# raimis/torchmd-net

Measured on AMD Instinct MI355X. Metric: molecules/sec (energy+force) ET-QM9, higher is better.
Workload: dtype fp32; 1 GPU; ET-QM9 energy+forces (TorchMD_Net derivative=True); model=equivariant-transformer, embedding_dimension=128, num_layers=8, num_rbf=64, num_heads=8, molecules_per_gpu=32, atoms_per_gpu=678, global_batch=32, parallelism=dp1, execution=hip-graph replay

## Files before the change

include/tmdnet.h:

```cpp
#ifndef TMDNET_H
#define TMDNET_H
#include <stddef.h>
#include <stdint.h>

#ifdef __cplusplus
extern "C" {
#endif

enum { TMDNET_OK = 0, TMDNET_BAD_ARGUMENT = 1, TMDNET_UNSUPPORTED = 2, TMDNET_LAUNCH_FAILED = 3,
       TMDNET_WORKSPACE_TOO_SMALL = 4 };
enum { TMDNET_F32 = 0, TMDNET_F64 = 1 };
enum { TMDNET_NL_BRUTE = 0, TMDNET_NL_SHARED = 1, TMDNET_NL_CELL = 2 };
enum { TMDNET_RBF_EXPNORM = 0, TMDNET_RBF_GAUSS = 1 };
enum { TMDNET_ACC_VEC_RESIDUAL = 1, TMDNET_ACC_EDGE = 2 };
enum { TMDNET_ACC_GRADS = 32 };
enum { TMDNET_ET_V_PLANAR = 4 };
enum { TMDNET_BWD2_ACC_EDGE = 8, TMDNET_BWD2_ACC_GVEC = 16 };
enum { TMDNET_ET_TWO_PASS = 64 };
enum { TMDNET_ACT_SILU = 0, TMDNET_ACT_SSP = 1, TMDNET_ACT_TANH = 2, TMDNET_ACT_SIGMOID = 3 };
#define TMDNET_ET_ACT(kv, attn) (((kv) << 8) | ((attn) << 12))

size_t tmdnet_nl_workspace_bytes(int n_atoms, int strategy, const double* box9, double cutoff_upper);
int tmdnet_nl_build(int dtype, int strategy, const void* pos, const int64_t* batch, int n_atoms,
                    const double* box9, int use_periodic, double cutoff_lower, double cutoff_upper,
                    int max_pairs, int loop, int include_transpose, int32_t* neighbors, void* deltas,
                    void* distances, int32_t* num_pairs, int32_t* row_ptr, int32_t* transpose_map,
                    int pad_output, void* workspace, size_t workspace_bytes, void* stream);
int tmdnet_nl_build_paired(int dtype, int strategy, const void* pos, const int64_t* batch, int n_atoms,
                           const double* box9, int use_periodic, double cutoff_lower, double cutoff_upper,
                           int max_pairs, int loop, int include_transpose, int32_t* neighbors, void* deltas,
                           void* distances, int32_t* num_pairs, int32_t* row_ptr, int32_t* transpose_map,
                           int pad_output, void* workspace, size_t workspace_bytes, int32_t* pair_row,
                           int32_t* pair_edge, int n_pair_slots, void* stream);

int tmdnet_nl_backward(int dtype, int n_atoms, const int32_t* row_ptr, const int32_t* transpose_map,
                       int max_pairs, const void* grad_deltas, const void* grad_distances,
                       const void* deltas, const void* distances, void* grad_pos, void* stream);
int tmdnet_nl_backward_multi(int dtype, int n_atoms, const int32_t* row_ptr, const int32_t* transpose_map,
                             int max_pairs, const void* grad_deltas, const void* grad_distances,
                             const void* grad_distances2, const void* deltas, const void* distances,
                             void* grad_pos, void* stream);

int tmdnet_nl_backward_edges(int dtype, int n_atoms, const int32_t* neighbors, int max_pairs,
                             const void* grad_deltas, const void* grad_distances, const void* deltas,
                             const void* distances, void* grad_pos, void* stream);

int tmdnet_nl_backward2(int dtype, int n_atoms, const int32_t* row_ptr, const int32_t* src,
                        const int32_t* transpose_map, int max_pairs, const void* grad_distances,
                        const void* deltas, const void* distances, const void* gg_pos, void* d_pos,
                        void* d_grad_deltas, void* d_grad_distances, void* stream);

int tmdnet_edge_geom_fwd(int dtype, int n_edges, int num_rbf, int rbf_type, const int32_t* src,
                         const int32_t* dst, const void* deltas, const void* dist, const void* mu,
                         const void* beta, double cutoff_lower, double cutoff_upper, void* rbf,
                         void* cutoff, void* unit, void* stream);
int tmdnet_edge_geom_fwd_rows(int dtype, int n_edges, int num_rbf, int rbf_type, const int32_t* src,
                              const int32_t* dst, const void* deltas, const void* dist, const void* mu,
                              const void* beta, double cutoff_lower, double cutoff_upper, void* rbf,
                              void* cutoff, void* unit, const int32_t* rows, int n_rows, void* rbf_rows,
                              void* stream);
int tmdnet_edge_geom_fwd_rows2(int dtype, int n_edges, int num_rbf, int rbf_type, const int32_t* src,
                               const int32_t* dst, const void* deltas, const void* dist, const void* mu,
                               const void* beta, double cutoff_lower, double cutoff_upper, void* rbf,
                               void* cutoff, void* unit, const int32_t* rows, int n_rows, void* rbf_rows,
                               void* drbf_rows, void* stream);
int tmdnet_edge_geom_bwd2(int dtype, int n_edges, int num_rbf, int rbf_type, const int32_t* src,
                          const int32_t* dst, const void* deltas, const void* dist, const void* mu,
                          const void* beta, double cutoff_lower, double cutoff_upper,
                          const void* grad_rbf, const void* grad_cutoff, const void* grad_unit,
                          const void* gg_deltas, const void* gg_dist, void* d_grad_rbf,
                          void* d_grad_cutoff, void* d_grad_unit, void* d_dist, void* d_deltas,
                          void* stream);
int tmdnet_rbf_deriv(int dtype, int num_rbf, int rbf_type, const void* dist, const void* mu,
                     const void* beta, double cutoff_lower, double cutoff_upper, const int32_t* rows,
                     int n_rows, void* out, void* stream);
int tmdnet_edge_geom_bwd(int dtype, int n_edges, int num_rbf, int rbf_type, const int32_t* src,
                         const int32_t* dst, const void* deltas, const void* dist, const void* mu,
                         const void* beta, double cutoff_lower, double cutoff_upper,
                         const void* grad_rbf, const void* grad_cutoff, const void* grad_unit,
                         void* grad_dist, void* grad_deltas, void* stream);
int tmdnet_edge_geom_bwd_multi(int dtype, int n_edges, int num_rbf, int rbf_type, const int32_t* src,
                               const int32_t* dst, const void* deltas, const void* dist, const void* mu,
                               const void* beta, double cutoff_lower, double cutoff_upper, const void* grad_rbf,
                               const void* grad_rbf2, const void* grad_rbf3, const void* grad_cutoff,
                               const void* grad_cutoff2, const void* grad_cutoff3, const void* grad_unit,
                               void* grad_dist, void* grad_deltas, void* stream);

int tmdnet_et_message_fwd(int dtype, int n_nodes, int hidden, int heads, const int32_t* row_ptr,
                          const int32_t* src, int max_pairs, const void* q, int ld_q, const void* k,
                          int ld_k, const void* v, int ld_v, const void* vec_in, const void* pk,
                          int ld_pk, const void* pv, int ld_pv, const void* cutoff, const void* unit,
                          void* x_out, void* vec_out, int flags, const int32_t* pk_rows,
                          const int32_t* order, void* stream);
#define TMDNET_TUNE_ET_BOTH_MAX_NODES 1
#define TMDNET_TUNE_ET_MERGED_MIN_NODES 2
int tmdnet_set_tuning(int key, int value);

int tmdnet_et_message_bwd(int dtype, int n_nodes, int hidden, int heads, const int32_t* row_ptr,
                          const int32_t* src, int max_pairs, const void* q, int ld_q, const void* k,
                          int ld_k, const void* v, int ld_v, const void* vec_in, const void* pk,
                          int ld_pk, const void* pv, int ld_pv, const void* cutoff, const void* unit,
// ... 150 lines not shown
#define TMDNET_TN_POST_O3 1
#define TMDNET_TN_POST_SO3 2
#define TMDNET_TN_RESID 3
#define TMDNET_TN_NORMS 4
#define TMDNET_TN_ENORM 5
#define TMDNET_TN_EOUT 6
int tmdnet_tn_node_fwd(int dtype, int op, int n_nodes, int hidden, const void* a, const void* b,
                       void* out, void* stream);
int tmdnet_tn_node_bwd(int dtype, int op, int n_nodes, int hidden, const void* a, const void* b,
                       const void* grad_out, const void* grad_add, void* ga, void* gb,
                       void* stream);
int tmdnet_tn_node_bwd2(int dtype, int op, int n_nodes, int hidden, const void* a, const void* b,
                        const void* grad_out, const void* t_a, const void* t_b, void* d_grad_out, void* d_a,
                        void* d_b, void* stream);

int tmdnet_silu_fwd(int dtype, int rows, int cols, const void* x, int ld_x, const void* row_scale,
                    void* out, void* stream);
int tmdnet_silu_bwd(int dtype, int rows, int cols, const void* x, int ld_x, const void* row_scale,
                    const void* grad_out, int ld_g, void* grad_x, void* grad_scale, void* stream);
int tmdnet_mlp2_up(int dtype, int rows, int cols, const void* pre, int ld_pre, const void* ghat, const void* a,
                   int ld_a, const void* gy, const void* scale, const void* sbar, void* ahat, void* dpre, void* dgy,
                   void* dscale, void* stream);
int tmdnet_mlp2_down(int dtype, int rows, int cols, const void* pre, int ld_pre, const void* dh, const void* dp,
                     void* c, void* stream);

int tmdnet_atom_sum_fwd(int dtype, int n_atoms, int n_mol, const void* x, const int64_t* batch,
                        const void* std_, const void* mean, void* y, void* stream);
int tmdnet_atom_sum_bwd(int dtype, int n_atoms, int n_mol, const void* grad_y, const int64_t* batch,
                        const void* std_, void* grad_x, void* stream);

int tmdnet_dot_sum_fwd(int dtype, int n_atoms, int K, const void* h, int ld_h, const void* w, const void* b0,
                       int n_mol, const int64_t* batch, const void* std_, const void* mean, void* y, void* stream);
int tmdnet_dot_sum_bwd(int dtype, int n_atoms, int K, const void* grad_y, const int64_t* batch, int n_mol,
                       const void* std_, const void* w, void* grad_h, void* stream);
int tmdnet_dot_sum_fwd_atoms(int dtype, int n_atoms, int K, const void* h, int ld_h, const void* w, const void* b0,
                             int n_mol, const int64_t* batch, const void* std_, const void* mean, void* atom_buf,
                             void* y, void* stream);

int tmdnet_layernorm_fwd_f32(int rows, int C, const void* x, int ldx, const void* w, const void* b, double eps,
                             void* y, int ldy, void* mean, void* rstd, void* stream);
int tmdnet_layernorm_bwd_f32(int rows, int C, const void* x, int ldx, const void* w, const void* mean,
                             const void* rstd, const void* grad_y, int ldg, void* grad_x, int accumulate,
                             void* stream);
int tmdnet_layernorm_bwd2_f32(int rows, int C, const void* x, int ldx, const void* w, const void* mean,
                              const void* rstd, const void* grad_y, int ldg, const void* t_gx, const void* t_gw,
                              const void* t_gb, void* d_grad_y, void* d_x, void* t_row, void* stream);
size_t tmdnet_layernorm_wgrad_workspace_bytes(int rows, int C);
int tmdnet_layernorm_wgrad_f32(int rows, int C, const void* x, int ldx, const void* mean, const void* rstd,
                               const void* grad_y, int ldg, void* grad_w, void* grad_b, void* workspace,
                               size_t workspace_bytes, void* stream);

size_t tmdnet_pair_index_workspace_bytes(int n_nodes);
int tmdnet_pair_index(int n_nodes, const int32_t* row_ptr, const int32_t* src, const int32_t* dst,
                      const int32_t* transpose, int max_pairs, const int32_t* num_pairs, int sorted_rows,
                      int32_t* pair_row, int32_t* pair_edge, int n_pair_slots, void* workspace,
                      size_t workspace_bytes, void* stream);

int tmdnet_gemm_f32(int n_problems, const int* dims, const void* const* ptrs, void* stream);
int tmdnet_gemm_ex_f32(int n_problems, const int* dims, const void* const* ptrs, void* stream);
int tmdnet_gemm_tn_f32(int n_problems, const int* dims, const void* const* ptrs, void* stream);
size_t tmdnet_gemm_tn_workspace_bytes(int n_problems, const int* dims);
int tmdnet_gemm_tn_f32_ws(int n_problems, const int* dims, const void* const* ptrs, void* workspace,
                          size_t workspace_bytes, void* stream);
int tmdnet_gemm_tn_rows_f32_ws(int n_problems, const int* dims, const void* const* ptrs, void* workspace,
                               size_t workspace_bytes, void* stream);
int tmdnet_embedding_fwd_f32(int n, int H, int num_types, const int64_t* z, int n_tables,
                             const void* const* tables, const int* ld_tables, void* const* outs,
                             const int* ld_outs, void* stream);
int tmdnet_embedding_bwd_f32(int n, int H, int num_types, const int64_t* z, int n_tables,
                             const void* const* grads, const int* ld_grads, void* const* outs, int accumulate,
                             void* stream);
int tmdnet_split_t_f32(int N, int K, const void* B, int ldb, void* Bp, void* stream);
int tmdnet_gemm_x3_f32(int M, int N, int K, const void* A, int lda, const void* Bp, const void* bias, void* C,
                       int ldc, int beta, void* stream);
int tmdnet_gemm_x3_ex_f32(int M, int N, int K, const void* A, int lda, const void* Bp, const void* bias, void* C,
                          int ldc, int beta, int act, void* pre, const void* rscale, const void* dpre, int ldx,
                          void* stream);
int tmdnet_gemm_x3w_f32(int M, int N, int K, const void* A, int lda, const void* W, int ldw, int trans_w,
                        const void* bias, void* C, int ldc, int beta, int act, void* pre, const void* rscale,
                        const void* dpre, int ldx, void* stream);
int tmdnet_proj_split_f32(int N, int K, const void* W, int ldw, void* Wp, void* stream);
int tmdnet_proj_f32(int M, int N, int K, const void* A, int lda, const void* Wp, long long piece_stride,
                    const void* bias, void* C, int ldc, void* stream);

size_t tmdnet_fep_image_bytes(int D, int R);
int tmdnet_fep_split_f32(int D, int R, const void* W, int ldw, const void* bias, void* img, void* wsc,
                         void* bias_out, void* stream);
size_t tmdnet_fep_frags_bytes(long long rows, int R);
int tmdnet_fep_frags_f32(long long rows, int R, const void* r_rows, const void* mu, const void* beta,
                         double cutoff_lower, double cutoff_upper, int rbf_type, void* frags, void* dscale,
                         void* stream);
int tmdnet_et_fused_fwd_f32(int n_nodes, int hidden, int heads, int num_rbf, const int32_t* row_ptr,
                            const int32_t* src, int max_pairs, const void* q, int ld_q, const void* k, int ld_k,
                            const void* v, int ld_v, const void* vec_in, const void* cutoff, const void* unit,
                            const int32_t* frag_rows, const void* frags, long long n_frag_rows, const void* img,
                            const void* wsc, const void* bias, void* x_out, void* vec_out, int flags, void* stream);

size_t tmdnet_et_fused_bwd_workspace_bytes(int max_pairs);
int tmdnet_et_fused_bwd_f32(int n_nodes, int hidden, int heads, int num_rbf, const int32_t* row_ptr,
                            const int32_t* src, int max_pairs, const void* q, int ld_q, const void* k, int ld_k,
                            const void* v, int ld_v, const void* vec_in, const void* cutoff, const void* unit,
                            const int32_t* frag_rows, const void* frags, const void* dscale, long long n_frag_rows,
                            const void* img, const void* wsc, const void* bias, const void* grad_x,
                            const void* grad_vec, void* gq, void* gk, void* gv, void* gvec_in, void* gcut,
                            void* gunit, void* gdist, int accumulate, void* workspace, size_t workspace_bytes,
                            void* stream);

int tmdnet_nbr_fused_fwd_f32(int n_nodes, int hidden, int num_rbf, const int32_t* row_ptr, const int32_t* src,
                             int max_pairs, const void* x, int ld_x, const void* cutoff, const int32_t* frag_rows,
                             const void* frags, long long n_frag_rows, const void* img, const void* wsc,
                             const void* bias, void* out, int ld_out, const void* x_self, void* out_self,
                             void* stream);
int tmdnet_nbr_fused_bwd_f32(int n_nodes, int hidden, int num_rbf, const int32_t* row_ptr, const int32_t* src,
                             int max_pairs, const void* x, int ld_x, const void* cutoff, const int32_t* frag_rows,
                             const void* frags, const void* dscale, long long n_frag_rows, const void* img,
                             const void* wsc, const void* bias, const void* grad_out, int ld_grad_out, void* gcut,
                             void* gdist, int accumulate, void* stream);

int tmdnet_mse2_fwd(int dtype, int n1, const void* a1, const void* b1, double w1, int n2, const void* a2,
                    const void* b2, double w2, void* out, void* stream);
int tmdnet_mse2_bwd(int dtype, int n1, const void* a1, const void* b1, double w1, int n2, const void* a2,
                    const void* b2, double w2, const void* grad_out, void* d1, void* d2, void* stream);

const char* tmdnet_build_info(void);

#ifdef __cplusplus
}
#endif
#endif
```

torchmd-net_amd/csrc/et_message.hip:

```cpp
#include <cstdlib>

#include "common.h"
#include "tmdnet.h"

namespace tmd {
namespace et {

template <typename T, int V> struct Vec;
template <> struct Vec<float, 1> { using t = float; };
template <> struct Vec<float, 2> { using t = float2; };
template <> struct Vec<float, 4> { using t = float4; };
template <> struct Vec<double, 1> { using t = double; };
template <> struct Vec<double, 2> { using t = double2; };
template <> struct Vec<double, 4> { using t = double4; };

template <typename T, int V> __device__ __forceinline__ void ldv(T (&o)[V], const T* p);
template <typename T, int V> __device__ __forceinline__ void ldv_(T (&o)[V], const T* p) {
  using VT = typename Vec<T, V>::t;
  const VT x = *reinterpret_cast<const VT*>(p);
  if constexpr (V == 1) { o[0] = x; }
  else if constexpr (V == 2) { o[0] = x.x; o[1] = x.y; }
  else { o[0] = x.x; o[1] = x.y; o[2] = x.z; o[3] = x.w; }
}
template <typename T, int V> __device__ __forceinline__ void ldv(T (&o)[V], const T* p) {
// ... 20 lines not shown
  if constexpr (V == 8) {
    T a[4], b[4];
#pragma unroll
    for (int i = 0; i < 4; ++i) { a[i] = o[i]; b[i] = o[4 + i]; }
    stv_<T, 4>(p, a);
    stv_<T, 4>(p + 4, b);
  } else {
    stv_<T, V>(p, o);
  }
}
template <typename T, int V> __device__ __forceinline__ void stv_acc(T* p, const T (&o)[V], bool acc) {
  if (acc) {
    T q[V];
    ldv<T, V>(q, p);
#pragma unroll
    for (int i = 0; i < V; ++i) q[i] += o[i];
    stv<T, V>(p, q);
  } else {
    stv<T, V>(p, o);
  }
}
template <typename T, int V> __device__ __forceinline__ void zero(T (&o)[V]) {
#pragma unroll
  for (int i = 0; i < V; ++i) o[i] = T(0);
}

template <typename T> struct Args {
  int n, H, d, L, lph, cap;
  int xcd;
  int HC;
  const int32_t* row_ptr;
  const int32_t* src;
  const int32_t* order;
  const T* q; int ldq;
  const T* k; int ldk;
  const T* v; int ldv;
  const T* vec;
  const T* pk; int ldpk;
  const T* pv; int ldpv;
  const int32_t* prow;
  const T* dpk;
  const T* dpv;
  T* gr;
  const T* C;
  const T* u;
  T* xo; T* veco;
  const T* gx; const T* gvec;
  T* gq; T* gk; T* gv; T* gveci; T* gpk; T* gpv; T* gC; T* gu;
  int acc;
  int planar;
  int vst;
  int act_kv;
  int act_at;
};

template <typename T, int V>
__device__ __forceinline__ void act(const T (&x)[V], bool has, T (&s)[V], T (&ds)[V], int code) {
  if (code == kActSilu) {
#pragma unroll
    for (int i = 0; i < V; ++i) {
      if (has) {
        Silu<T> f(x[i]);
        s[i] = f.s;
        ds[i] = f.d(x[i]);
      } else {
        s[i] = T(1);
        ds[i] = T(0);
      }
    }
    return;
  }
#pragma unroll
  for (int i = 0; i < V; ++i) {
    if (has) {
      ActF<T> f(x[i], code);
      s[i] = f.s;
      ds[i] = f.d(x[i]);
    } else {
      s[i] = T(1);
      ds[i] = T(0);
    }
  }
}
template <typename T> __device__ __forceinline__ const T* opt(const T* p, size_t off, const T* dummy) {
  return p ? p + off : dummy;
}


__device__ __forceinline__ int xcd_block(int b, int nwg, int xcd) { return xcd ? xcd_remap(b, nwg) : b; }
struct Geo {
  int node;
  int sub;
  int es;
  int el;
  int cg;
};

template <int S, int CS, bool ORD, int WPB = 4>
__device__ __forceinline__ Geo geo(int n, int L, const int32_t* order, int xcd, int blk, int nwg) {
  Geo g;
  const int wid = threadIdx.x >> 6;
  const int npb = WPB / S;
  const int nbn = (n + npb - 1) / npb;
  const int lb = xcd_block(blk, nwg, xcd);
  g.cg = CS > 1 ? __builtin_amdgcn_readfirstlane(lb / nbn) : 0;
  const int w = __builtin_amdgcn_readfirstlane((CS > 1 ? lb % nbn : lb) * npb + wid / S);
  g.sub = __builtin_amdgcn_readfirstlane(wid % S);
  g.node = w < n ? (ORD ? __builtin_amdgcn_readfirstlane(order[w]) : w) : -1;
  const int lane = lane_id();
  g.es = lane / L;
  g.el = lane % L;
  return g;
}

template <typename T, int V> __device__ __forceinline__ void xor_slots(T (&a)[V], int L) {
  for (int o = L; o < TMD_WAVE; o <<= 1)
#pragma unroll
    for (int i = 0; i < V; ++i) a[i] += __shfl_xor(a[i], o);
}

template <typename T, int S, int NV>
__device__ __forceinline__ void reduce_waves(T (&a)[NV], int sub, T* lds) {
  if constexpr (S > 1) {
    const int wid = threadIdx.x >> 6, lane = lane_id();
    const int base = (wid - sub) * 64 * NV;
    if (sub > 0) {
#pragma unroll
      for (int i = 0; i < NV; ++i) lds[base + (sub * NV + i) * 64 + lane] = a[i];
    }
    __syncthreads();
    if (sub == 0) {
#pragma unroll
      for (int s2 = 1; s2 < S; ++s2)
#pragma unroll
        for (int i = 0; i < NV; ++i) a[i] += lds[base + (s2 * NV + i) * 64 + lane];
    }
  }
}

template <typename T, int S, int PD, typename St, typename LD, typename F>
__device__ __forceinline__ void edge_chunks_pf(const Args<T>& A, int b, int e, int EPW, const Geo& G,
                                               LD&& ld, F&& body) {
  const int lane = lane_id();
  St cur, nxt, nx2;
  const int step = EPW * S;
  for (int c = b; c < e; c += TMD_WAVE) {
    const int n = min(TMD_WAVE, e - c);
    int s_r = 0, p_r = c + lane;
    T C_r = T(0), u0_r = T(0), u1_r = T(0), u2_r = T(0);
    if (lane < n) {
      const int k = c + lane;
      s_r = A.src[k];
      TMD_DCHECK(s_r >= 0 && s_r < A.n);
      if (A.prow) p_r = A.prow[k];
      C_r = A.C[k];
      u0_r = A.u[3 * k];
      u1_r = A.u[3 * k + 1];
      u2_r = A.u[3 * k + 2];
    }
    int j0 = EPW * G.sub;
    if (j0 < n) {
      ld(__shfl(p_r, min(j0 + G.es, n - 1)), cur);
      if constexpr (PD == 2) ld(__shfl(p_r, min(j0 + step + G.es, n - 1)), nxt);
    }
    for (; j0 < n; j0 += step) {
      const int j = j0 + G.es;
      const int jj = j < n ? j : n - 1;
      const int s = __shfl(s_r, jj);
      const T Ce = __shfl(C_r, jj), u0 = __shfl(u0_r, jj), u1 = __shfl(u1_r, jj), u2 = __shfl(u2_r, jj);
      const int kn = __shfl(p_r, min(j0 + PD * step + G.es, n - 1));
      auto pre = [&]() { ld(kn, PD == 2 ? nx2 : nxt); };
      if (j < n) body(c + j, s, Ce, u0, u1, u2, cur, pre);
      else pre();
      cur = nxt;
      if constexpr (PD == 2) nxt = nx2;
    }
  }
}

template <typename T, int S, typename F>
__device__ __forceinline__ void edge_chunks(const Args<T>& A, int b, int e, int EPW, const Geo& G, F&& body) {
  const int lane = lane_id();
  const int step = EPW * S;
  for (int c = b; c < e; c += TMD_WAVE) {
    const int n = min(TMD_WAVE, e - c);
    int s_r = 0, p_r = c + lane;
    T C_r = T(0), u0_r = T(0), u1_r = T(0), u2_r = T(0);
    if (lane < n) {
      const int k = c + lane;
      s_r = A.src[k];
      TMD_DCHECK(s_r >= 0 && s_r < A.n);
      if (A.prow) p_r = A.prow[k];
      C_r = A.C[k];
      u0_r = A.u[3 * k];
      u1_r = A.u[3 * k + 1];
      u2_r = A.u[3 * k + 2];
    }
    for (int j0 = EPW * G.sub; j0 < n; j0 += step) {
      const int j = j0 + G.es;
      const int jj = j < n ? j : n - 1;
      const int s = __shfl(s_r, jj), row = __shfl(p_r, jj);
      const T Ce = __shfl(C_r, jj), u0 = __shfl(u0_r, jj), u1 = __shfl(u1_r, jj), u2 = __shfl(u2_r, jj);
      if (j < n) body(c + j, s, Ce, u0, u1, u2, row);
    }
  }
}

template <typename T, int V, int S, int CS, bool ORD, bool GA = true>
__global__ __launch_bounds__(256) void k_fwd(Args<T> A) {
  const int AKV = GA ? A.act_kv : kActSilu, AAT = GA ? A.act_at : kActSilu;
  __shared__ T lds[S > 1 ? 4 * 64 * 4 * V : 1];
  const Geo G = geo<S, CS, ORD>(A.n, A.L, A.order, A.xcd, blockIdx.x, gridDim.x);
  const int t = G.node;
  const bool on = true;
  const int EPW = TMD_WAVE / A.L;
  const int c0 = G.cg * A.HC + G.el * V;
  const int hh = c0 / A.d, cc = c0 % A.d;
  const int vo = A.planar ? c0 : hh * 3 * A.d + cc;
  const bool hk = A.pk != nullptr, hv = A.pv != nullptr, hw = A.vec != nullptr;
  const int pvd = hv ? A.vst : 0, vcd = hw ? A.H : 0;
  (void)vcd;
  T ax[V], a0[V], a1[V], a2[V];
  zero(ax); zero(a0); zero(a1); zero(a2);
  if (t >= 0) {
    T q[V];
    ldv<T, V>(q, A.q + (size_t)t * A.ldq + c0);
    const int b = min(A.row_ptr[t], A.cap), e = min(A.row_ptr[t + 1], A.cap);
    const T* dummy = A.q + (size_t)t * A.ldq;
    struct St { T k[V], x[V], a[V], b[V]; };
    auto ld = [&](int k, St& st) {
      ldv<T, V>(st.k, opt(A.pk, (size_t)k * A.ldpk + c0, dummy + c0));
      const T* pvs = opt(A.pv, (size_t)k * A.ldpv + vo, dummy);
      ldv<T, V>(st.x, pvs);
      ldv<T, V>(st.a, pvs + pvd);
      ldv<T, V>(st.b, pvs + 2 * pvd);
    };
    auto body = [&](int k, int s, T Ce, T u0, T u1, T u2, const St& st, auto&& pre) {
      (void)k;
      T kk[V], vx[V], v1[V], v2[V], w0[V], w1[V], w2[V];
      ldv<T, V>(kk, A.k + (size_t)s * A.ldk + c0);
      const T* vs = A.v + (size_t)s * A.ldv + vo;
      ldv<T, V>(vx, vs);
      ldv<T, V>(v1, vs + A.vst);
      ldv<T, V>(v2, vs + 2 * A.vst);
      const T* vecs = hw ? A.vec + (size_t)s * 3 * A.H + c0 : dummy + c0;
      ldv<T, V>(w0, vecs);
      ldv<T, V>(w1, vecs + vcd);
      ldv<T, V>(w2, vecs + 2 * vcd);
      pre();
      if (!hw) { zero(w0); zero(w1); zero(w2); }
      T dk[V], dvx[V], dv1[V], dv2[V], dd[V];
      act<T, V>(st.k, hk, dk, dd, AKV);
      act<T, V>(st.x, hv, dvx, dd, AKV);
      act<T, V>(st.a, hv, dv1, dd, AKV);
      act<T, V>(st.b, hv, dv2, dd, AKV);
      T part = T(0);
#pragma unroll
      for (int i = 0; i < V; ++i) part += q[i] * kk[i] * dk[i];
      part = group_sum(part, A.lph);
      const ActF<T> sa(part, AAT);
      const T a = sa.s * Ce;
#pragma unroll
      for (int i = 0; i < V; ++i) {
        ax[i] += vx[i] * dvx[i] * a;
        const T v1e = v1[i] * dv1[i], v2e = v2[i] * dv2[i];
        a0[i] += w0[i] * v1e + v2e * u0;
        a1[i] += w1[i] * v1e + v2e * u1;
        a2[i] += w2[i] * v1e + v2e * u2;
      }
    };
    edge_chunks_pf<T, S, 1, St>(A, b, e, EPW, G, ld, body);
  }
  xor_slots(ax, A.L); xor_slots(a0, A.L); xor_slots(a1, A.L); xor_slots(a2, A.L);
  T all[4 * V];
#pragma unroll
  for (int i = 0; i < V; ++i) { all[i] = ax[i]; all[V + i] = a0[i]; all[2 * V + i] = a1[i]; all[3 * V + i] = a2[i]; }
  reduce_waves<T, S, 4 * V>(all, G.sub, lds);
  if (t >= 0 && G.sub == 0 && on && G.es == 0) {
#pragma unroll
    for (int i = 0; i < V; ++i) { ax[i] = all[i]; a0[i] = all[V + i]; a1[i] = all[2 * V + i]; a2[i] = all[3 * V + i]; }
    stv<T, V>(A.xo + (size_t)t * A.H + c0, ax);
    T* vo_ = A.veco + (size_t)t * 3 * A.H + c0;
    stv<T, V>(vo_, a0);
    stv<T, V>(vo_ + A.H, a1);
    stv<T, V>(vo_ + 2 * A.H, a2);
  }
}

template <typename T>
__device__ __forceinline__ void zero_pad_rows(const Args<T>& A, int blk, int nwg) {
  const int e0 = min(A.row_ptr[A.n], A.cap);
  if (e0 >= A.cap) return;
  const long long rows = A.cap - e0;
  const long long tid = (long long)blk * blockDim.x + threadIdx.x, nth = (long long)nwg * blockDim.x;
  if (A.gpk) {
    for (long long i = tid; i < rows * A.H; i += nth)
      A.gpk[(size_t)(e0 + i / A.H) * A.ldpk + i % A.H] = T(0);
  }
  if (A.gpv) {
    const int w = 3 * A.H;
    for (long long i = tid; i < rows * w; i += nth)
      A.gpv[(size_t)(e0 + i / w) * A.ldpv + i % w] = T(0);
  }
  if (A.gC)
    for (long long i = tid; i < rows; i += nth) A.gC[e0 + i] = T(0);
  if (A.gu)
    for (long long i = tid; i < rows * 3; i += nth) A.gu[3 * (size_t)e0 + i] = T(0);
  if (A.gr)
    for (long long i = tid; i < rows; i += nth) A.gr[e0 + i] = T(0);
}

template <typename T, int V, int S, int CS, bool DR, bool AG = false, bool GA = true>
__device__ __forceinline__ void bwd_dst_body(const Args<T>& A, int blk, int nwg) {
  const int AKV = GA ? A.act_kv : kActSilu, AAT = GA ? A.act_at : kActSilu;
  __shared__ T lds[S > 1 ? 4 * 64 * V : 1];
  const Geo G = geo<S, CS, false>(A.n, A.L, nullptr, A.xcd, blk, nwg);
  const int t = G.node;
  const bool on = true;
  const int EPW = TMD_WAVE / A.L;
  const int c0 = G.cg * A.HC + G.el * V;
  const int hh = c0 / A.d, cc = c0 % A.d;
  const int vo = A.planar ? c0 : hh * 3 * A.d + cc;
  const bool hk = A.pk != nullptr, hv = A.pv != nullptr, hw = A.vec != nullptr;
  const int pvd = hv ? A.vst : 0, vcd = hw ? A.H : 0;
  (void)vcd;
  const bool head_leader = on && (G.el % A.lph) == 0;
  T gq[V];
  zero(gq);
  if (t >= 0) {
    T q[V], gx[V], g0[V], g1[V], g2[V];
    ldv<T, V>(q, A.q + (size_t)t * A.ldq + c0);
    ldv<T, V>(gx, A.gx + (size_t)t * A.H + c0);
    const T* gvt = A.gvec + (size_t)t * 3 * A.H + c0;
    ldv<T, V>(g0, gvt);
    ldv<T, V>(g1, gvt + A.H);
    ldv<T, V>(g2, gvt + 2 * A.H);
    const int b = min(A.row_ptr[t], A.cap), e = min(A.row_ptr[t + 1], A.cap);
    const T* dummy = A.q + (size_t)t * A.ldq;
    const bool acc_edge = (A.acc & TMDNET_ACC_EDGE) && G.el == 0;
    struct St { T k[V], x[V], a[V], b[V]; int row; };
    auto ld = [&](int k, St& st) {
      ldv<T, V>(st.k, opt(A.pk, (size_t)k * A.ldpk + c0, dummy + c0));
      const T* pvs = opt(A.pv, (size_t)k * A.ldpv + vo, dummy);
      ldv<T, V>(st.x, pvs);
      ldv<T, V>(st.a, pvs + pvd);
      ldv<T, V>(st.b, pvs + 2 * pvd);
      st.row = k;
    };
    auto body = [&](int k, int s, T Ce, T u0, T u1, T u2, const St& st, auto&& pre) {
      T oc = T(0), ou0 = T(0), ou1 = T(0), ou2 = T(0), orr = T(0);
      if (acc_edge) {
        oc = A.gC[k];
        ou0 = A.gu[3 * k];
        ou1 = A.gu[3 * k + 1];
        ou2 = A.gu[3 * k + 2];
        if constexpr (DR) orr = A.gr[k];
      }
      T kk[V], vx[V], v1[V], v2[V], w0[V], w1[V], w2[V];
      ldv<T, V>(kk, A.k + (size_t)s * A.ldk + c0);
      const T* vs = A.v + (size_t)s * A.ldv + vo;
      ldv<T, V>(vx, vs);
      ldv<T, V>(v1, vs + A.vst);
      ldv<T, V>(v2, vs + 2 * A.vst);
      const T* vecs = hw ? A.vec + (size_t)s * 3 * A.H + c0 : dummy + c0;
      ldv<T, V>(w0, vecs);
      ldv<T, V>(w1, vecs + vcd);
      ldv<T, V>(w2, vecs + 2 * vcd);
      T ik[AG ? V : 1], ix[AG ? V : 1], i1[AG ? V : 1], i2[AG ? V : 1];
      if constexpr (AG) {
        if (hk) ldv<T, V>(ik, A.gpk + (size_t)k * A.ldpk + c0); else zero(ik);
        if (hv) {
          const T* gp = A.gpv + (size_t)k * A.ldpv + vo;
          ldv<T, V>(ix, gp); ldv<T, V>(i1, gp + A.vst); ldv<T, V>(i2, gp + 2 * A.vst);
        } else {
          zero(ix); zero(i1); zero(i2);
        }
      }
      T dpk_[DR ? V : 1], dpx_[DR ? V : 1], dp1_[DR ? V : 1], dp2_[DR ? V : 1];
      if constexpr (DR) {
        ldv<T, V>(dpk_, opt(A.dpk, (size_t)st.row * A.ldpk + c0, dummy + c0));
        const T* dps = opt(A.dpv, (size_t)st.row * A.ldpv + vo, dummy);
        ldv<T, V>(dpx_, dps);
        ldv<T, V>(dp1_, dps + pvd);
        ldv<T, V>(dp2_, dps + 2 * pvd);
      }
      pre();
      if (!hw) { zero(w0); zero(w1); zero(w2); }
      const T (&pk)[V] = st.k;
      const T (&px)[V] = st.x;
      const T (&p1)[V] = st.a;
      const T (&p2)[V] = st.b;
      T dk[V], ddk[V], dvx[V], dv1[V], dv2[V], ddx[V], dd1[V], dd2[V];
      act<T, V>(pk, hk, dk, ddk, AKV);
      act<T, V>(px, hv, dvx, ddx, AKV);
      act<T, V>(p1, hv, dv1, dd1, AKV);
      act<T, V>(p2, hv, dv2, dd2, AKV);
      T part = T(0), ga = T(0), gu0 = T(0), gu1 = T(0), gu2 = T(0);
#pragma unroll
      for (int i = 0; i < V; ++i) {
        part += q[i] * kk[i] * dk[i];
        ga += gx[i] * vx[i] * dvx[i];
        const T v2e = v2[i] * dv2[i];
        gu0 += g0[i] * v2e;
        gu1 += g1[i] * v2e;
        gu2 += g2[i] * v2e;
      }
      part = group_sum(part, A.lph);
      ga = group_sum(ga, A.lph);
      const ActF<T> sa(part, AAT);
      const T a = sa.s * Ce;
      const T gs = ga * Ce * sa.d(part);
      T gpk[V], gpx[V], gp1[V], gp2[V];
#pragma unroll
      for (int i = 0; i < V; ++i) {
        gq[i] += gs * kk[i] * dk[i];
        gpk[i] = gs * q[i] * kk[i] * ddk[i];
        gpx[i] = gx[i] * a * vx[i] * ddx[i];
        const T gv1e = g0[i] * w0[i] + g1[i] * w1[i] + g2[i] * w2[i];
        gp1[i] = gv1e * v1[i] * dd1[i];
        const T gv2e = g0[i] * u0 + g1[i] * u1 + g2[i] * u2;
        gp2[i] = gv2e * v2[i] * dd2[i];
      }
      const T gc = group_sum(head_leader ? ga * sa.s : T(0), A.L);
      gu0 = group_sum(gu0, A.L);
      gu1 = group_sum(gu1, A.L);
      gu2 = group_sum(gu2, A.L);
      T grr = T(0);
      if constexpr (DR) {
#pragma unroll
        for (int i = 0; i < V; ++i)
          grr += (hk ? gpk[i] * dpk_[i] : T(0)) +
                 (hv ? gpx[i] * dpx_[i] + gp1[i] * dp1_[i] + gp2[i] * dp2_[i] : T(0));
        grr = group_sum(grr, A.L);
        if (on && (A.gpk || A.gpv)) {
          if (hk && A.gpk) stv<T, V>(A.gpk + (size_t)k * A.ldpk + c0, gpk);
          if (hv && A.gpv) {
            T* gp = A.gpv + (size_t)k * A.ldpv + vo;
            stv<T, V>(gp, gpx);
            stv<T, V>(gp + A.vst, gp1);
            stv<T, V>(gp + 2 * A.vst, gp2);
          }
        }
      } else {
        if (on) {
          if constexpr (AG) {
#pragma unroll
            for (int i = 0; i < V; ++i) { gpk[i] += ik[i]; gpx[i] += ix[i]; gp1[i] += i1[i]; gp2[i] += i2[i]; }
          }
          const bool ag = !AG && (A.acc & TMDNET_ACC_GRADS);
          if (hk) stv_acc<T, V>(A.gpk + (size_t)k * A.ldpk + c0, gpk, ag);
          if (hv) {
            T* gp = A.gpv + (size_t)k * A.ldpv + vo;
            stv_acc<T, V>(gp, gpx, ag);
            stv_acc<T, V>(gp + A.vst, gp1, ag);
            stv_acc<T, V>(gp + 2 * A.vst, gp2, ag);
          }
        }
      }
      if (G.el == 0) {
        A.gC[k] = oc + gc;
        A.gu[3 * k] = ou0 + gu0;
        A.gu[3 * k + 1] = ou1 + gu1;
        A.gu[3 * k + 2] = ou2 + gu2;
        if constexpr (DR) A.gr[k] = orr + grr;
      }
    };
    edge_chunks_pf<T, S, 1, St>(A, b, e, EPW, G, ld, body);
  }
  xor_slots(gq, A.L);
  reduce_waves<T, S, V>(gq, G.sub, lds);
  if (t >= 0 && G.sub == 0 && on && G.es == 0)
    stv_acc<T, V>(A.gq + (size_t)t * A.ldq + c0, gq, A.acc & TMDNET_ACC_GRADS);
  zero_pad_rows(A, blk, nwg);
}

template <typename T, int V, int S, int CS, bool GA = true>
__device__ __forceinline__ void bwd_src_body(const Args<T>& A, int blk, int nwg) {
  const int AKV = GA ? A.act_kv : kActSilu, AAT = GA ? A.act_at : kActSilu;
  __shared__ T lds[S > 1 ? 4 * 64 * 7 * V : 1];
  const Geo G = geo<S, CS, false>(A.n, A.L, nullptr, A.xcd, blk, nwg);
  const int j = G.node;
  const bool on = true;
  const int EPW = TMD_WAVE / A.L;
  const int c0 = G.cg * A.HC + G.el * V;
  const int hh = c0 / A.d, cc = c0 % A.d;
  const int vo = A.planar ? c0 : hh * 3 * A.d + cc;
  const bool hk = A.pk != nullptr, hv = A.pv != nullptr, hw = A.vec != nullptr;
  const int pvd = hv ? A.vst : 0, vcd = hw ? A.H : 0;
  (void)vcd;
  T gk[V], gvx[V], gv1[V], gv2[V], gw0[V], gw1[V], gw2[V];
  zero(gk); zero(gvx); zero(gv1); zero(gv2); zero(gw0); zero(gw1); zero(gw2);
  if (j >= 0) {
    T kk[V], vx[V], v1[V], v2[V], w0[V], w1[V], w2[V];
    ldv<T, V>(kk, A.k + (size_t)j * A.ldk + c0);
    const T* vj = A.v + (size_t)j * A.ldv + vo;
    ldv<T, V>(vx, vj);
    ldv<T, V>(v1, vj + A.vst);
    ldv<T, V>(v2, vj + 2 * A.vst);
    if (hw) {
      const T* vecj = A.vec + (size_t)j * 3 * A.H + c0;
      ldv<T, V>(w0, vecj);
      ldv<T, V>(w1, vecj + A.H);
      ldv<T, V>(w2, vecj + 2 * A.H);
    } else {
      zero(w0); zero(w1); zero(w2);
    }
    const int b = min(A.row_ptr[j], A.cap), e = min(A.row_ptr[j + 1], A.cap);
    const T* dummy = A.k + (size_t)j * A.ldk;
    struct St { T k[V], x[V], a[V], b[V]; };
    auto ld = [&](int k, St& st) {
      ldv<T, V>(st.k, opt(A.pk, (size_t)k * A.ldpk + c0, dummy + c0));
      const T* pvs = opt(A.pv, (size_t)k * A.ldpv + vo, dummy);
      ldv<T, V>(st.x, pvs);
      ldv<T, V>(st.a, pvs + pvd);
      ldv<T, V>(st.b, pvs + 2 * pvd);
    };
    auto body = [&](int k, int m, T Ce, T u0, T u1, T u2, const St& st, auto&& pre) {
      u0 = -u0; u1 = -u1; u2 = -u2;
      (void)k;
      T qm[V], gxm[V], g0[V], g1[V], g2[V];
      ldv<T, V>(qm, A.q + (size_t)m * A.ldq + c0);
      ldv<T, V>(gxm, A.gx + (size_t)m * A.H + c0);
      const T* gvm = A.gvec + (size_t)m * 3 * A.H + c0;
      ldv<T, V>(g0, gvm);
      ldv<T, V>(g1, gvm + A.H);
      ldv<T, V>(g2, gvm + 2 * A.H);
      pre();
      const T (&pk)[V] = st.k;
      const T (&px)[V] = st.x;
      const T (&p1)[V] = st.a;
      const T (&p2)[V] = st.b;
      T dk[V], ddk[V], dvx[V], dv1[V], dv2[V], dd[V];
      act<T, V>(pk, hk, dk, ddk, AKV);
      act<T, V>(px, hv, dvx, dd, AKV);
      act<T, V>(p1, hv, dv1, dd, AKV);
      act<T, V>(p2, hv, dv2, dd, AKV);
      T part = T(0), ga = T(0);
#pragma unroll
      for (int i = 0; i < V; ++i) {
        part += qm[i] * kk[i] * dk[i];
        ga += gxm[i] * vx[i] * dvx[i];
      }
      part = group_sum(part, A.lph);
      ga = group_sum(ga, A.lph);
      const ActF<T> sa(part, AAT);
      const T a = sa.s * Ce;
      const T gs = ga * Ce * sa.d(part);
#pragma unroll
      for (int i = 0; i < V; ++i) {
        gk[i] += gs * qm[i] * dk[i];
        gvx[i] += gxm[i] * a * dvx[i];
        const T gv1e = g0[i] * w0[i] + g1[i] * w1[i] + g2[i] * w2[i];
        gv1[i] += gv1e * dv1[i];
        const T gv2e = g0[i] * u0 + g1[i] * u1 + g2[i] * u2;
        gv2[i] += gv2e * dv2[i];
        const T v1e = v1[i] * dv1[i];
        gw0[i] += g0[i] * v1e;
        gw1[i] += g1[i] * v1e;
        gw2[i] += g2[i] * v1e;
      }
    };
    edge_chunks_pf<T, S, 1, St>(A, b, e, EPW, G, ld, body);
  }
  xor_slots(gk, A.L); xor_slots(gvx, A.L); xor_slots(gv1, A.L); xor_slots(gv2, A.L); xor_slots(gw0, A.L); xor_slots(gw1, A.L); xor_slots(gw2, A.L);
  T all[7 * V];
#pragma unroll
  for (int i = 0; i < V; ++i) {
    all[i] = gk[i]; all[V + i] = gvx[i]; all[2 * V + i] = gv1[i]; all[3 * V + i] = gv2[i];
    all[4 * V + i] = gw0[i]; all[5 * V + i] = gw1[i]; all[6 * V + i] = gw2[i];
  }
  reduce_waves<T, S, 7 * V>(all, G.sub, lds);
  if (j >= 0 && G.sub == 0 && on && G.es == 0) {
#pragma unroll
    for (int i = 0; i < V; ++i) {
      gk[i] = all[i]; gvx[i] = all[V + i]; gv1[i] = all[2 * V + i]; gv2[i] = all[3 * V + i];
      gw0[i] = all[4 * V + i]; gw1[i] = all[5 * V + i]; gw2[i] = all[6 * V + i];
    }
    const bool ag = A.acc & TMDNET_ACC_GRADS;
    stv_acc<T, V>(A.gk + (size_t)j * A.ldk + c0, gk, ag);
    T* gvj = A.gv + (size_t)j * A.ldv + vo;
    stv_acc<T, V>(gvj, gvx, ag);
    stv_acc<T, V>(gvj + A.vst, gv1, ag);
    stv_acc<T, V>(gvj + 2 * A.vst, gv2, ag);
    if (A.gveci != nullptr) {
      if (A.acc & TMDNET_ACC_VEC_RESIDUAL) {
        const T* gr = A.gvec + (size_t)j * 3 * A.H + c0;
        T r0[V], r1[V], r2[V];
        ldv<T, V>(r0, gr);
        ldv<T, V>(r1, gr + A.H);
        ldv<T, V>(r2, gr + 2 * A.H);
#pragma unroll
        for (int i = 0; i < V; ++i) { gw0[i] += r0[i]; gw1[i] += r1[i]; gw2[i] += r2[i]; }
      }
      T* gwj = A.gveci + (size_t)j * 3 * A.H + c0;
      stv_acc<T, V>(gwj, gw0, ag);
      stv_acc<T, V>(gwj + A.H, gw1, ag);
      stv_acc<T, V>(gwj + 2 * A.H, gw2, ag);
    }
  }
}

template <typename T, int V, bool DR>
constexpr int bwd_min_waves() { return (DR && sizeof(T) == 4 && V <= 4) ? 3 : 1; }

template <typename T, int V, int S, int CS, bool DR, bool AG = false, bool GA = true>
__global__ __launch_bounds__(256, (bwd_min_waves<T, V, DR>())) void k_bwd_dst(Args<T> A) {
  bwd_dst_body<T, V, S, CS, DR, AG, GA>(A, blockIdx.x, gridDim.x);
}
template <typename T, int V, int S, int CS, bool GA = true>
__global__ __launch_bounds__(256) void k_bwd_src(Args<T> A) {
  bwd_src_body<T, V, S, CS, GA>(A, blockIdx.x, gridDim.x);
}
template <typename T, int V, int S, int CS, bool DR, bool AG = false, bool GA = true>
__global__ __launch_bounds__(256, (bwd_min_waves<T, V, DR>())) void k_bwd_both(Args<T> A) {
  const int split = (int)gridDim.x / 2;
  if ((int)blockIdx.x < split) bwd_dst_body<T, V, S, CS, DR, AG, GA>(A, blockIdx.x, split);
  else bwd_src_body<T, V, S, CS, GA>(A, blockIdx.x - split, split);
}

template <typename T, int V, int S, int PD, bool GA = true>
__device__ __forceinline__ void bwd_merged_body(const Args<T>& A, int blk, int nwg) {
  const int AKV = GA ? A.act_kv : kActSilu, AAT = GA ? A.act_at : kActSilu;
  constexpr int NA = 8 * V;
  extern __shared__ __attribute__((aligned(16))) char dyn_lds[];
  T* lds = reinterpret_cast<T*>(dyn_lds);
  const int HM = A.H;
  const Geo G = geo<S, 1, false>(A.n, A.L, nullptr, A.xcd, blk, nwg);
  const int t = G.node;
  const int EPW = TMD_WAVE / A.L;
  const int c0 = G.el * V;
  const int hh = c0 / A.d, cc = c0 % A.d;
  const int vo = A.planar ? c0 : hh * 3 * A.d + cc;
  const bool hk = A.pk != nullptr, hv = A.pv != nullptr, hw = A.vec != nullptr;
  const int pvd = hv ? A.vst : 0, vcd = hw ? A.H : 0;
  const bool head_leader = (G.el % A.lph) == 0;
  T* nv = lds + ((threadIdx.x >> 6) / S) * 12 * HM;
  if (t >= 0 && G.sub == 0 && G.es == 0) {
    T a[V];
    const T* src[12];
    const T* gvt = A.gvec + (size_t)t * 3 * A.H;
    const T* vt = A.v + (size_t)t * A.ldv;
    const T* wt = A.vec + (size_t)t * 3 * A.H;
    src[0] = A.q + (size_t)t * A.ldq + c0; src[1] = A.gx + (size_t)t * A.H + c0;
    src[2] = gvt + c0; src[3] = gvt + A.H + c0; src[4] = gvt + 2 * A.H + c0;
    src[5] = A.k + (size_t)t * A.ldk + c0;
    src[6] = vt + vo; src[7] = vt + vo + A.vst; src[8] = vt + vo + 2 * A.vst;
    src[9] = hw ? wt + c0 : src[0]; src[10] = hw ? wt + A.H + c0 : src[0]; src[11] = hw ? wt + 2 * A.H + c0 : src[0];
#pragma unroll
    for (int r = 0; r < 12; ++r) {
      ldv<T, V>(a, src[r]);
      if (r >= 9 && !hw) zero(a);
      stv<T, V>(nv + r * HM + c0, a);
    }
  }
  __syncthreads();
  T gq[V], gk[V], gvx[V], gv1[V], gv2[V], gw0[V], gw1[V], gw2[V];
  zero(gq); zero(gk); zero(gvx); zero(gv1); zero(gv2); zero(gw0); zero(gw1); zero(gw2);
  if (t >= 0) {
    const int b = min(A.row_ptr[t], A.cap), e = min(A.row_ptr[t + 1], A.cap);
    const T* dummy = A.q + (size_t)t * A.ldq;
    const bool acc_edge = (A.acc & TMDNET_ACC_EDGE) && G.el == 0;
    struct St { T k[V], x[V], a[V], b[V]; int row; };
    auto ld = [&](int k, St& st) {
      ldv<T, V>(st.k, opt(A.pk, (size_t)k * A.ldpk + c0, dummy + c0));
      const T* pvs = opt(A.pv, (size_t)k * A.ldpv + vo, dummy);
      ldv<T, V>(st.x, pvs);
      ldv<T, V>(st.a, pvs + pvd);
      ldv<T, V>(st.b, pvs + 2 * pvd);
      st.row = k;
    };
    auto body = [&](int k, int s, T Ce, T u0, T u1, T u2, const St& st, auto&& pre) {
      T oc = T(0), ou0 = T(0), ou1 = T(0), ou2 = T(0), orr = T(0);
      if (acc_edge) {
        oc = A.gC[k]; ou0 = A.gu[3 * k]; ou1 = A.gu[3 * k + 1]; ou2 = A.gu[3 * k + 2]; orr = A.gr[k];
      }
      T kk[V], vx[V], v1[V], v2[V], w0[V], w1[V], w2[V], qs[V], gxs[V], h0[V], h1[V], h2[V];
      ldv<T, V>(kk, A.k + (size_t)s * A.ldk + c0);
      const T* vs = A.v + (size_t)s * A.ldv + vo;
      ldv<T, V>(vx, vs);
      ldv<T, V>(v1, vs + A.vst);
      ldv<T, V>(v2, vs + 2 * A.vst);
      const T* vecs = hw ? A.vec + (size_t)s * 3 * A.H + c0 : dummy + c0;
      ldv<T, V>(w0, vecs);
      ldv<T, V>(w1, vecs + vcd);
      ldv<T, V>(w2, vecs + 2 * vcd);
      ldv<T, V>(qs, A.q + (size_t)s * A.ldq + c0);
      ldv<T, V>(gxs, A.gx + (size_t)s * A.H + c0);
      const T* gvs = A.gvec + (size_t)s * 3 * A.H + c0;
      ldv<T, V>(h0, gvs);
      ldv<T, V>(h1, gvs + A.H);
      ldv<T, V>(h2, gvs + 2 * A.H);
      T dpk_[V], dpx_[V], dp1_[V], dp2_[V];
      ldv<T, V>(dpk_, opt(A.dpk, (size_t)st.row * A.ldpk + c0, dummy + c0));
      const T* dps = opt(A.dpv, (size_t)st.row * A.ldpv + vo, dummy);
      ldv<T, V>(dpx_, dps);
      ldv<T, V>(dp1_, dps + pvd);
      ldv<T, V>(dp2_, dps + 2 * pvd);
      pre();
      if (!hw) { zero(w0); zero(w1); zero(w2); }
      T dk[V], ddk[V], dvx[V], dv1[V], dv2[V], ddx[V], dd1[V], dd2[V];
// ... 608 lines not shown
    if (A.dC) {
#pragma unroll
      for (int u = 0; u < NB_U; ++u) dc[u] = wave_sum(on ? dc[u] : T(0));
      if (lane == 0) {
#pragma unroll
        for (int u = 0; u < NB_U; ++u)
          if (sq[u] >= 0) A.dC[k0 + u] = dc[u];
      }
    }
  });
  if (on && A.dgout) stv<T, V>(A.dgout + (size_t)t * A.H + c0, acc);
}

template <typename T, int V>
__global__ __launch_bounds__(256) void k_nb_bwd2_src(NbArgs<T> A) {
  const int j = blockIdx.x * (blockDim.x / TMD_WAVE) + threadIdx.x / TMD_WAVE;
  if (j >= A.n) return;
  const int lane = lane_id();
  const bool on = lane < A.L;
  const int c0 = on ? lane * V : 0;
  T acc[V];
  zero(acc);
  nb_edges(A, j, [&](int k0, const int (&sq)[NB_U], const T (&cq)[NB_U]) {
    T gm[NB_U][V], wk[NB_U][V], gwk[NB_U][V], ck[NB_U], gck[NB_U];
#pragma unroll
    for (int u = 0; u < NB_U; ++u) {
      const int kt = sq[u] >= 0 ? A.tr[k0 + u] : -1;
      const bool live = kt >= 0 && sq[u] != j;
      const int m = live ? sq[u] : j;
      const int k = live ? kt : k0;
      TMD_DCHECK(!live || k < A.cap);
      ldv<T, V>(gm[u], A.gout + (size_t)m * A.ldg + c0);
      ldv<T, V>(wk[u], A.w + (size_t)k * A.ldw + c0);
      if (A.ggw) ldv<T, V>(gwk[u], A.ggw + (size_t)k * A.H + c0); else zero(gwk[u]);
      ck[u] = live ? A.C[k] : T(0);
      gck[u] = (live && A.ggC) ? A.ggC[k] : T(0);
    }
#pragma unroll
    for (int u = 0; u < NB_U; ++u)
#pragma unroll
      for (int i = 0; i < V; ++i) acc[i] += gm[u][i] * (gwk[u][i] * ck[u] + gck[u] * wk[u][i]);
  });
  if (on) stv<T, V>(A.dx + (size_t)j * A.H + c0, acc);
}

static inline int pick_vec(int H) {
  if (H % 256 == 0) return 4;
  if (H % 128 == 0) return 2;
  return 1;
}

template <typename T>
static bool aligned(const void* p, int ld, int V) {
  if (!p) return true;
  return ((uintptr_t)p % (sizeof(T) * V)) == 0 && (ld % V) == 0;
}

template <typename T, template <typename, int> class K, typename AT>
static int launch_v(int V, int n, AT A, hipStream_t st) {
  const int tb = 256, wpb = tb / TMD_WAVE;
  dim3 g((n + wpb - 1) / wpb);
  if (n <= 0) return kOk;
  if (V == 1) hipLaunchKernelGGL((K<T, 1>::fn), g, dim3(tb), 0, st, A);
  else if (V == 2) hipLaunchKernelGGL((K<T, 2>::fn), g, dim3(tb), 0, st, A);
  else hipLaunchKernelGGL((K<T, 4>::fn), g, dim3(tb), 0, st, A);
  return hipGetLastError() == hipSuccess ? kOk : kLaunchFailed;
}

static inline int et_waves_per_node(int n, int bytes_per_lane_vec) {
  if (bytes_per_lane_vec > 32) return 1;
  static const int env_s = [] { const char* e = getenv("TMDNET_ET_S"); return e ? atoi(e) : 0; }();
  if (env_s > 0) return env_s >= 4 ? 4 : env_s >= 2 ? 2 : 1;
  if (n < 4096) return 4;
  if (n < 8192) return 2;
  return 1;
}

template <typename T, int V, int S, int KIND, bool ORD, bool GA>
static int et_launch_k(const Args<T>& A, dim3 g, dim3 b, int nbn, hipStream_t st);

template <typename T, int V, int S, int KIND, bool ORD>
static int et_launch_vs(Args<T> A, hipStream_t st) {
  int cs = 1;
  if (KIND == 1 || A.H % (cs * V) || (A.H / cs / V) & (A.H / cs / V - 1) || A.H / cs / V < A.lph ||
      A.H / cs / V > 64)
    cs = 1;
  A.HC = A.H / cs;
  A.L = A.HC / V;
  if (A.L > 64 || (A.L & (A.L - 1))) return kUnsupported;
  const int nbn = (A.n + (4 / S) - 1) / (4 / S);
  const dim3 g(nbn * cs), b(256);
  if (A.act_kv == kActSilu && A.act_at == kActSilu)
    return et_launch_k<T, V, S, KIND, ORD, false>(A, g, b, nbn, st);
  return et_launch_k<T, V, S, KIND, ORD, true>(A, g, b, nbn, st);
}

template <typename T, int V, int S, int KIND, bool ORD, bool GA>
static int et_launch_k(const Args<T>& A, dim3 g, dim3 b, int nbn, hipStream_t st) {
  if (KIND == 0) hipLaunchKernelGGL((k_fwd<T, V, S, 1, ORD, GA>), g, b, 0, st, A);
  else if (KIND == 1) hipLaunchKernelGGL((k_bwd_dst<T, V, S, 1, false, false, GA>), g, b, 0, st, A);
  else if (KIND == 2) hipLaunchKernelGGL((k_bwd_src<T, V, S, 1, GA>), g, b, 0, st, A);
  else if (KIND == 3) hipLaunchKernelGGL((k_bwd_both<T, V, S, 1, false, false, GA>), dim3(2 * nbn), b, 0, st, A);
  else if (KIND == 4) hipLaunchKernelGGL((k_bwd_dst<T, V, S, 1, true, false, GA>), g, b, 0, st, A);
  else if (KIND == 5) hipLaunchKernelGGL((k_bwd_both<T, V, S, 1, true, false, GA>), dim3(2 * nbn), b, 0, st, A);
  else if (KIND == 6) hipLaunchKernelGGL((k_bwd_both<T, V, S, 1, false, true, GA>), dim3(2 * nbn), b, 0, st, A);
  else if (KIND == 8 || KIND == 9) {
    const size_t node = (size_t)(4 / S) * 12 * A.H, red = S > 1 ? 4 * 64 * 8 * V : 1;
    const size_t bytes = (node > red ? node : red) * sizeof(T);
    if (KIND == 8) hipLaunchKernelGGL((k_bwd_merged<T, V, S, 1, GA>), dim3(nbn), b, bytes, st, A);
    else hipLaunchKernelGGL((k_bwd_merged<T, V, S, 0, GA>), dim3(nbn), b, bytes, st, A);
  }
  else hipLaunchKernelGGL((k_bwd_dst<T, V, S, 1, false, true, GA>), g, b, 0, st, A);
  return hipGetLastError() == hipSuccess ? kOk : kLaunchFailed;
}

static constexpr int kBwdFuseNodes = 16384;

static int g_tune[3] = {-1, -1, -1};
static int tune_get(int key) {
  int& v = g_tune[key];
  if (v < 0) {
    const char* e = getenv(key == TMDNET_TUNE_ET_BOTH_MAX_NODES ? "TMDNET_ET_FUSE" : "TMDNET_ET_MERGED_MIN");
    v = e ? atoi(e) : kBwdFuseNodes;
  }
  return v;
}

template <typename T, int V, int KIND, bool ORD>
static int et_launch_v(const Args<T>& A, hipStream_t st) {
  int S = et_waves_per_node(A.n, (int)sizeof(T) * V);
  static const bool env_s_set = getenv("TMDNET_ET_S") != nullptr;
  if (KIND == 0 && !env_s_set && (int)sizeof(T) * V <= 32) S = 4;
  static const int bwd_s = getenv("TMDNET_ET_BWD_S") ? atoi(getenv("TMDNET_ET_BWD_S")) : 0;
  if (KIND != 0 && bwd_s && (int)sizeof(T) * V <= 32) S = bwd_s >= 4 ? 4 : bwd_s >= 2 ? 2 : 1;
  if (S == 4) return et_launch_vs<T, V, (sizeof(T) * V <= 32 ? 4 : 1), KIND, ORD>(A, st);
  if (S == 2) return et_launch_vs<T, V, (sizeof(T) * V <= 32 ? 2 : 1), KIND, ORD>(A, st);
  return et_launch_vs<T, V, 1, KIND, ORD>(A, st);
}

template <typename T, int KIND, bool ORD>
static int et_launch(int V, const Args<T>& A, hipStream_t st) {
  if (A.n <= 0) return kOk;
  switch (V) {
    case 1: return et_launch_v<T, 1, KIND, ORD>(A, st);
    case 2: return et_launch_v<T, 2, KIND, ORD>(A, st);
    case 4: return et_launch_v<T, 4, KIND, ORD>(A, st);
    case 8: return et_launch_v<T, 8, KIND, ORD>(A, st);
  }
  return kUnsupported;
}

template <typename T, int V> struct KNbFwd { static constexpr auto fn = k_nb_fwd<T, V>; };
template <typename T, int V> struct KNbDst { static constexpr auto fn = k_nb_bwd_dst<T, V>; };
template <typename T, int V> struct KNbSrc { static constexpr auto fn = k_nb_bwd_src<T, V>; };
template <typename T, int V> struct KNb2Dst { static constexpr auto fn = k_nb_bwd2_dst<T, V>; };
template <typename T, int V> struct KNb2Src { static constexpr auto fn = k_nb_bwd2_src<T, V>; };

template <typename T>
static int setup(Args<T>& A, int n, int H, int heads, const int32_t* row_ptr, const int32_t* src,
                 int cap, const void* q, int ldq, const void* k, int ldk, const void* v, int ldv_,
                 const void* vec, const void* pk, int ldpk, const void* pv, int ldpv, const void* C,
                 const void* u, const int32_t* order, int& V, const int32_t* prow = nullptr) {
  if (H <= 0 || heads <= 0 || H % heads) return kBadArgument;
  if (H % 32 == 0) V = H / 32;
  else if (H < 32) V = 1;
  else return kUnsupported;

  if (V != 1 && V != 2 && V != 4 && V != 8) return kUnsupported;
  const int d = H / heads;
  if (d % V) return kUnsupported;
  const int lph = d / V;
  if (lph & (lph - 1)) return kUnsupported;
  const int VA = V > 4 ? 4 : V;
  if (!aligned<T>(q, ldq, VA) || !aligned<T>(k, ldk, VA) || !aligned<T>(v, ldv_, VA) ||
      !aligned<T>(pk, ldpk, VA) || !aligned<T>(pv, ldpv, VA) || !aligned<T>(vec, H, VA))
    return kBadArgument;
  A = Args<T>{};
  A.n = n; A.H = H; A.d = d; A.L = H / V; A.HC = H; A.lph = lph; A.cap = cap;
  A.planar = 0; A.vst = d;
  A.row_ptr = row_ptr; A.src = src; A.order = order;
  A.xcd = 1;
  A.q = (const T*)q; A.ldq = ldq; A.k = (const T*)k; A.ldk = ldk; A.v = (const T*)v; A.ldv = ldv_;
  A.vec = (const T*)vec; A.pk = (const T*)pk; A.ldpk = ldpk; A.pv = (const T*)pv; A.ldpv = ldpv;
  A.prow = prow;
  A.C = (const T*)C; A.u = (const T*)u;
  return kOk;
}

template <typename T>
static int set_acts(Args<T>& A, int flags) {
  A.act_kv = (flags >> 8) & 15;
  A.act_at = (flags >> 12) & 15;
  return (A.act_kv > kActSigmoid || A.act_at > kActSigmoid) ? kBadArgument : kOk;
}

template <typename T>
static int fwd(int n, int H, int heads, const int32_t* row_ptr, const int32_t* src, int cap,
               const void* q, int ldq, const void* k, int ldk, const void* v, int ldv_,
               const void* vec, const void* pk, int ldpk, const void* pv, int ldpv, const void* C,
               const void* u, void* xo, void* veco, int flags, const int32_t* prow, const int32_t* order,
               hipStream_t st) {
  Args<T> A;
  int V;
  int rc = setup<T>(A, n, H, heads, row_ptr, src, cap, q, ldq, k, ldk, v, ldv_, vec, pk, ldpk, pv,
                    ldpv, C, u, order, V, prow);
  if (rc) return rc;
  if ((rc = set_acts(A, flags))) return rc;
  if (flags & TMDNET_ET_V_PLANAR) { A.planar = 1; A.vst = H; }
  A.xo = (T*)xo;
  A.veco = (T*)veco;
  return order ? et_launch<T, 0, true>(V, A, st) : et_launch<T, 0, false>(V, A, st);
}

template <typename T>
static int bwd(int n, int H, int heads, const int32_t* row_ptr, const int32_t* src, int cap,
               const void* q, int ldq, const void* k, int ldk, const void* v, int ldv_,
               const void* vec, const void* pk, int ldpk, const void* pv, int ldpv, const void* C,
               const void* u, const void* gx, const void* gvec, void* gq, void* gk, void* gv,
               void* gveci, void* gpk, void* gpv, void* gC, void* gu, const void* dpk, const void* dpv,
               void* gr, int acc, const int32_t* prow, const int32_t* order, hipStream_t st) {
  Args<T> A;
  int V;
  int rc = setup<T>(A, n, H, heads, row_ptr, src, cap, q, ldq, k, ldk, v, ldv_, vec, pk, ldpk, pv,
                    ldpv, C, u, order, V, prow);
  if (rc) return rc;
  A.gx = (const T*)gx; A.gvec = (const T*)gvec;
  A.gq = (T*)gq; A.gk = (T*)gk; A.gv = (T*)gv; A.gveci = (T*)gveci;
  A.gpk = (T*)gpk; A.gpv = (T*)gpv; A.gC = (T*)gC; A.gu = (T*)gu;
  A.dpk = (const T*)dpk; A.dpv = (const T*)dpv; A.gr = (T*)gr;
  A.acc = acc;
  if ((rc = set_acts(A, acc))) return rc;
  static const int bwd_v = getenv("TMDNET_ET_BWD_V") ? atoi(getenv("TMDNET_ET_BWD_V")) : 0;
  if (bwd_v && bwd_v < V && H % (32 * bwd_v) == 0 && H / bwd_v <= 64 && (A.d / bwd_v) > 0 &&
      A.d % bwd_v == 0 && !((A.d / bwd_v) & (A.d / bwd_v - 1))) {
    V = bwd_v;
    A.lph = A.d / V;
  }
  if (acc & TMDNET_ET_V_PLANAR) { A.planar = 1; A.vst = H; }
  const bool dr = gr != nullptr;
  if (dr && ((A.pk && !dpk) || (A.pv && !dpv))) return kBadArgument;
  if (!dr && ((A.pk && !gpk) || (A.pv && !gpv))) return kBadArgument;
  const int fuse_nodes = tune_get(TMDNET_TUNE_ET_BOTH_MAX_NODES);
  const bool ag = !dr && (acc & TMDNET_ACC_GRADS) && (A.pk || A.pv);
  static const int merged = getenv("TMDNET_ET_MERGED") ? atoi(getenv("TMDNET_ET_MERGED")) : 1;
  const int merged_min = tune_get(TMDNET_TUNE_ET_MERGED_MIN_NODES);
  if (dr && merged && n >= merged_min && !(acc & TMDNET_ET_TWO_PASS) && !A.gpk && !A.gpv)
    return merged == 2 ? et_launch<T, 9, false>(V, A, st) : et_launch<T, 8, false>(V, A, st);
  if (n < fuse_nodes)
    return dr ? et_launch<T, 5, false>(V, A, st) : ag ? et_launch<T, 6, false>(V, A, st) : et_launch<T, 3, false>(V, A, st);
  rc = dr ? et_launch<T, 4, false>(V, A, st) : ag ? et_launch<T, 7, false>(V, A, st) : et_launch<T, 1, false>(V, A, st);
  if (rc) return rc;
  return et_launch<T, 2, false>(V, A, st);
}

struct Bwd2Ex {
  int ldggq, ldggk, ldggv, ldoq, ldok, ldov, ldopk, ldopv;
  const int32_t* tr;
  void* scratch;
  const int32_t* prow;
  const void* ggsc;
};

template <typename T>
static int bwd2(int n, int H, int heads, const int32_t* row_ptr, const int32_t* src, int cap,
                const void* q, int ldq, const void* k, int ldk, const void* v, int ldv_,
                const void* vec, const void* pk, int ldpk, const void* pv, int ldpv, const void* C,
                const void* u, const void* gx, const void* gvec, const void* ggq, const void* ggk,
                const void* ggv, const void* ggw, const void* ggpk, int ldggpk, const void* ggpv,
                int ldggpv, const void* ggC, const void* ggu, void* o_gx, void* o_gvec, void* o_q,
                void* o_k, void* o_v, void* o_vec, void* o_pk, void* o_pv, void* o_C, void* o_u,
                int flags, hipStream_t st, const Bwd2Ex* ex = nullptr) {
  Args2<T> B{};
  int V;
  int rc = setup<T>(B.a, n, H, heads, row_ptr, src, cap, q, ldq, k, ldk, v, ldv_, vec, pk, ldpk, pv,
                    ldpv, C, u, nullptr, V);
  if (rc) return rc;
  if (H % 64 == 0) V = H / 64;
  const int d = H / heads;
  if ((V != 1 && V != 2 && V != 4) || d % V || ((d / V) & (d / V - 1))) return kUnsupported;
  B.a.L = H / V;
  B.a.lph = d / V;
  if (B.a.L > 64 || (B.a.L & (B.a.L - 1))) return kUnsupported;
  if (!aligned<T>(ggpk, ldggpk, V) || !aligned<T>(ggpv, ldggpv, V)) return kBadArgument;
  if ((rc = set_acts(B.a, flags))) return rc;
  if (flags & TMDNET_ET_V_PLANAR) { B.a.planar = 1; B.a.vst = H; }
  B.a.gx = (const T*)gx; B.a.gvec = (const T*)gvec;
  B.ggq = (const T*)ggq; B.ggk = (const T*)ggk; B.ggv = (const T*)ggv; B.ggw = (const T*)ggw;
  B.ggpk = (const T*)ggpk; B.ldggpk = ldggpk; B.ggpv = (const T*)ggpv; B.ldggpv = ldggpv;
  B.ggC = (const T*)ggC; B.ggu = (const T*)ggu;
  B.o_gx = (T*)o_gx; B.o_gvec = (T*)o_gvec; B.o_q = (T*)o_q; B.o_k = (T*)o_k; B.o_v = (T*)o_v;
  B.o_vec = (T*)o_vec; B.o_pk = (T*)o_pk; B.o_pv = (T*)o_pv; B.o_C = (T*)o_C; B.o_u = (T*)o_u;
  B.ldggq = B.ldok = B.ldoq = H; B.ldggk = H; B.ldggv = B.ldov = 3 * H; B.ldopk = H; B.ldopv = 3 * H;
  if (ex) {
    auto pick = [](int x, int dflt) { return x ? x : dflt; };
    B.ldggq = pick(ex->ldggq, H); B.ldggk = pick(ex->ldggk, H); B.ldggv = pick(ex->ldggv, 3 * H);
    B.ldoq = pick(ex->ldoq, H); B.ldok = pick(ex->ldok, H); B.ldov = pick(ex->ldov, 3 * H);
    B.ldopk = pick(ex->ldopk, H); B.ldopv = pick(ex->ldopv, 3 * H);
    if (B.ldggq < H || B.ldggk < H || B.ldggv < 3 * H || B.ldoq < H || B.ldok < H || B.ldov < 3 * H ||
        B.ldopk < H || B.ldopv < 3 * H)
      return kBadArgument;
    if (!aligned<T>(ggq, B.ldggq, V) || !aligned<T>(ggk, B.ldggk, V) || !aligned<T>(ggv, B.ldggv, V) ||
        !aligned<T>(o_q, B.ldoq, V) || !aligned<T>(o_pk, B.ldopk, V) || !aligned<T>(o_pv, B.ldopv, V))
      return kBadArgument;
    if ((ex->tr == nullptr) != (ex->scratch == nullptr)) return kBadArgument;
    if (ex->scratch) {
      if (H % 4 || B.ldok % 4 || B.ldov % 4 || ((uintptr_t)o_k % (4 * sizeof(T))) ||
          ((uintptr_t)o_v % (4 * sizeof(T))) || ((uintptr_t)ex->scratch % (4 * sizeof(T))))
        return kBadArgument;
      B.tr = ex->tr;
      B.o_src = (T*)ex->scratch;
    }
    B.a.prow = ex->prow;
    if (ex->ggsc && !ex->prow) return kBadArgument;
    B.ggsc = (const T*)ex->ggsc;
  }
  B.acc_edge = (flags & TMDNET_BWD2_ACC_EDGE) ? 1 : 0;
  B.acc_gvec = (flags & TMDNET_BWD2_ACC_GVEC) ? 1 : 0;
  if (n <= 0) return kOk;
  static const int s_env = getenv("TMDNET_BWD2_S") ? atoi(getenv("TMDNET_BWD2_S")) : 0;
  int S = n < 2048 ? 8 : (n < 4096 ? 4 : (n < 8192 ? 2 : 1));
  if (s_env == 1 || s_env == 2 || s_env == 4 || s_env == 8) S = s_env;
  if (S == 8 && V != 2) S = 4;
  const dim3 g(S == 8 ? n : (n + 4 / S - 1) / (4 / S)), b(S == 8 ? 512 : 256);
#define TMD_L2(VV, SS) hipLaunchKernelGGL((k_bwd2<T, VV, SS>), g, b, 0, st, B)
  if (V == 1) { if (S == 4) TMD_L2(1, 4); else if (S == 2) TMD_L2(1, 2); else TMD_L2(1, 1); }
// ... 227 lines not shown
```

torchmd-net_amd/csrc/gemm.hip:

```cpp
#include <cstdio>
#include <cstdlib>

#include "common.h"
#include "tmdnet.h"

namespace tmd {
namespace gemm {

struct Prob {
  int M, N, K, lda, ldb, ldc, trans_b, beta;
  const float* A;
  const float* B;
  const float* bias;
  float* C;
  int tiles_n, tile0;
  int act, ldx;
  float* pre;
  const float* rscale;
  const float* dpre;
};

struct Group {
  Prob p[4];
  int n;
// ... 633 lines not shown
__global__ __launch_bounds__(256) void k_proj_split(int N, int K, const float* W, int ldw, unsigned short* Wp) {
  const int i = blockIdx.x * 256 + threadIdx.x;
  if (i >= N * K / 4) return;
  const int n = i / (K / 4), k = (i % (K / 4)) * 4;
  const float4 v = *reinterpret_cast<const float4*>(W + (size_t)n * ldw + k);
  const float x[4] = {v.x, v.y, v.z, v.w};
  unsigned h[4], m[4], l[4];
#pragma unroll
  for (int j = 0; j < 4; ++j) split3(x[j], h[j], m[j], l[j]);
  const size_t o = (size_t)n * K + k, ps = (size_t)N * K;
  *reinterpret_cast<uint2*>(Wp + o) = make_uint2((h[0] >> 16) | h[1], (h[2] >> 16) | h[3]);
  *reinterpret_cast<uint2*>(Wp + ps + o) = make_uint2((m[0] >> 16) | m[1], (m[2] >> 16) | m[3]);
  *reinterpret_cast<uint2*>(Wp + 2 * ps + o) = make_uint2((l[0] >> 16) | l[1], (l[2] >> 16) | l[3]);
}

template <int KS, int MB, int BN>
__global__ __launch_bounds__(256) void k_proj_x3(Args P) {
  constexpr int K = 32 * KS, LD = K + 8;
  __shared__ __attribute__((aligned(16))) unsigned short w[3][BN][LD];
  __shared__ __attribute__((aligned(16))) float sb[BN];
  const int lane = threadIdx.x & 63, wave = threadIdx.x >> 6;
  const int n0 = blockIdx.x * BN;
  const int m0 = (blockIdx.y * 4 + wave) * (16 * MB);
  const int nr = min(BN, P.N - n0);
  const int kq = 8 * (lane >> 4);
  float4 ar[MB][KS][2];
#pragma unroll
  for (int mb = 0; mb < MB; ++mb) {
    const float* r = P.A + (size_t)min(m0 + 16 * mb + (lane & 15), P.M - 1) * P.lda + kq;
#pragma unroll
    for (int ks = 0; ks < KS; ++ks) {
      ar[mb][ks][0] = *reinterpret_cast<const float4*>(r + 32 * ks);
      ar[mb][ks][1] = *reinterpret_cast<const float4*>(r + 32 * ks + 4);
    }
  }
  constexpr int CH = K / 8;
  constexpr int NL = (3 * BN * CH + 255) / 256;
  u4 stg[NL];
#pragma unroll
  for (int i = 0; i < NL; ++i) {
    const int c = threadIdx.x + 256 * i;
    const int p = c / (BN * CH), rc = c % (BN * CH), n = rc / CH, k = (rc % CH) * 8;
    if (c < 3 * BN * CH)
      stg[i] = *reinterpret_cast<const u4*>(P.Wp + p * P.pstride + (size_t)min(n0 + n, P.N - 1) * K + k);
  }
#pragma unroll
  for (int i = 0; i < NL; ++i) {
    const int c = threadIdx.x + 256 * i;
    const int p = c / (BN * CH), rc = c % (BN * CH), n = rc / CH, k = (rc % CH) * 8;
    if (c < 3 * BN * CH) *reinterpret_cast<u4*>(&w[p][n][k]) = stg[i];
  }
  if (threadIdx.x < BN) sb[threadIdx.x] = P.bias ? P.bias[min(n0 + (int)threadIdx.x, P.N - 1)] : 0.f;
  bf8 a[MB][KS][3];
#pragma unroll
  for (int mb = 0; mb < MB; ++mb)
#pragma unroll
    for (int ks = 0; ks < KS; ++ks) split8(ar[mb][ks][0], ar[mb][ks][1], a[mb][ks]);
  __syncthreads();
  if (m0 >= P.M) return;
  for (int nb = 0; nb < nr; nb += 16) {
    bf8 b[KS][3];
#pragma unroll
    for (int ks = 0; ks < KS; ++ks)
#pragma unroll
      for (int p = 0; p < 3; ++p)
        b[ks][p] = *reinterpret_cast<const bf8*>(&w[p][nb + (lane & 15)][32 * ks + kq]);
    f4 acc[MB];
#pragma unroll
    for (int mb = 0; mb < MB; ++mb) acc[mb] = f4{0.f, 0.f, 0.f, 0.f};
    constexpr int TW[6] = {2, 1, 0, 1, 0, 0}, TA[6] = {0, 1, 2, 0, 1, 0};
#pragma unroll
    for (int t = 0; t < 6; ++t)
#pragma unroll
      for (int ks = 0; ks < KS; ++ks)
#pragma unroll
        for (int mb = 0; mb < MB; ++mb)
          acc[mb] = __builtin_amdgcn_mfma_f32_16x16x32_bf16(b[ks][TW[t]], a[mb][ks][TA[t]], acc[mb], 0, 0, 0);
    const int nl = nb + 4 * (lane >> 4);
    const f4 bv = *reinterpret_cast<const f4*>(&sb[nl]);
#pragma unroll
    for (int mb = 0; mb < MB; ++mb) {
      const int m = m0 + 16 * mb + (lane & 15);
      if (m < P.M) *reinterpret_cast<f4*>(P.C + (size_t)m * P.ldc + n0 + nl) = acc[mb] + bv;
    }
  }
}

__global__ __launch_bounds__(256) void k_split_t(int N, int K, const float* B, int ldb, unsigned short* Bp) {
  const int i = blockIdx.x * 256 + threadIdx.x;
  if (i >= N * (K / 4)) return;
  const int k = (i / N) * 4, n = i % N;
  const float x[4] = {B[(size_t)k * ldb + n], B[(size_t)(k + 1) * ldb + n], B[(size_t)(k + 2) * ldb + n],
                      B[(size_t)(k + 3) * ldb + n]};
  unsigned h[4], m[4], l[4];
#pragma unroll
  for (int j = 0; j < 4; ++j) split3(x[j], h[j], m[j], l[j]);
  const size_t o = (size_t)n * K + k, ps = (size_t)N * K;
  *reinterpret_cast<uint2*>(Bp + o) = make_uint2((h[0] >> 16) | h[1], (h[2] >> 16) | h[3]);
  *reinterpret_cast<uint2*>(Bp + ps + o) = make_uint2((m[0] >> 16) | m[1], (m[2] >> 16) | m[3]);
  *reinterpret_cast<uint2*>(Bp + 2 * ps + o) = make_uint2((l[0] >> 16) | l[1], (l[2] >> 16) | l[3]);
}

struct XArgs {
  int M, N, K, lda, ldc, beta;
  int nx, ny, remap;
  const float* A;
  const unsigned short* Bp;
  const float* bias;
  float* C;
  int act, ldx;
  float* pre;
  const float* rscale;
  const float* dpre;
  const float* W;
  int ldw;
};
template <int MB, int BN, int PD, int WS = 0>
__global__ __launch_bounds__(256) void k_gemm_x3(XArgs P) {
  constexpr int KC = BN >= 128 ? 64 : 128, LD = KC + 8, NB = BN / 16, SPC = KC / 32;
  __shared__ __attribute__((aligned(16))) unsigned short w[3][BN][LD];
  const int lane = threadIdx.x & 63, wave = threadIdx.x >> 6;
  int bx = blockIdx.x, by = blockIdx.y;
  if (P.remap) {
    const int T = P.nx * P.ny, b = blockIdx.x, x = b & 7, q = T >> 3, r = T & 7;
    const int t = x * q + min(x, r) + (b >> 3);
    bx = t % P.nx;
    by = t / P.nx;
  }
  const int n0 = bx * BN;
  const int m0 = (by * 4 + wave) * (16 * MB);
  const int kq = 8 * (lane >> 4);
  const size_t ps = (size_t)P.N * P.K;
  f4 acc[NB][MB];
#pragma unroll
  for (int nb = 0; nb < NB; ++nb)
#pragma unroll
    for (int mb = 0; mb < MB; ++mb) acc[nb][mb] = f4{0.f, 0.f, 0.f, 0.f};
  const float* arow[MB];
#pragma unroll
  for (int mb = 0; mb < MB; ++mb) arow[mb] = P.A + (size_t)min(m0 + 16 * mb + (lane & 15), P.M - 1) * P.lda + kq;
  const int nks_all = P.K / 32;
  float4 an[PD][MB][2];
#pragma unroll
  for (int d = 0; d < PD; ++d)
#pragma unroll
    for (int mb = 0; mb < MB; ++mb) {
      const int ko = 32 * min(d, nks_all - 1);
      an[d][mb][0] = *reinterpret_cast<const float4*>(arow[mb] + ko);
      an[d][mb][1] = *reinterpret_cast<const float4*>(arow[mb] + ko + 4);
    }
  constexpr int TW[6] = {2, 1, 0, 1, 0, 0}, TA[6] = {0, 1, 2, 0, 1, 0};
  for (int s0 = 0; s0 < nks_all; s0 += PD) {
#pragma unroll
    for (int d = 0; d < PD; ++d) {
      const int st_ = s0 + d;
      if (st_ < nks_all) {
        if (st_ % SPC == 0) {
          const int kc = 32 * st_;
          const int nks = min(KC, P.K - kc) / 32;
          constexpr int CH = KC / 8, NL = 3 * BN * CH / 256;
          const int ch = nks * 4;
          if constexpr (WS == 0) {
            u4 stg[NL];
#pragma unroll
            for (int i = 0; i < NL; ++i) {
              const int c = threadIdx.x + 256 * i;
// ... 777 lines not shown
  gemm::GroupTN G{};
  int tiles = 0, kmax = 0;
  const int rc = tn_group(n_problems, dims, ptrs, np, G, tiles, kmax);
  if (rc != kOk) return rc;
  float* ws = (float*)workspace;
  if (ws && workspace_bytes < tmdnet_gemm_tn_workspace_bytes(n_problems, dims)) return kWorkspaceTooSmall;
  launch_tn(G, tiles, kmax, ws, (hipStream_t)stream);
  return hipGetLastError() == hipSuccess ? kOk : kLaunchFailed;
}

extern "C" int tmdnet_gemm_tn_f32(int n_problems, const int* dims, const void* const* ptrs, void* stream) {
  return gemm_tn(n_problems, dims, ptrs, 5, nullptr, 0, stream);
}

extern "C" size_t tmdnet_gemm_tn_workspace_bytes(int n_problems, const int* dims) {
  if (n_problems < 1 || n_problems > gemm::TN_MAX || !dims) return 0;
  int tiles = 0, kmax = 0;
  for (int i = 0; i < n_problems; ++i) {
    const int* d = dims + 12 * i;
    tiles += ((d[0] + 31) / 32) * ((d[1] + 31) / 32);
    kmax = max(kmax, d[2] + d[3]);
  }
  TNShape sh[gemm::TN_MAX];
  for (int i = 0; i < n_problems; ++i) {
    const int* d = dims + 12 * i;
    sh[i] = TNShape{d[0], (d[10] || d[11]) ? d[1] - 1 : d[1], d[2] + d[3]};
  }
  int Sv[gemm::TN_MAX], nt[gemm::TN_MAX];
  long long p0[gemm::TN_MAX], parts = 0;
  tn_plan_v(n_problems, sh, true, Sv, nt, p0, parts);
  const int S = tn_split(tiles, kmax);
  const size_t b32 = S > 1 ? sizeof(float) * 1024 * (size_t)tiles * S : 0;
  const size_t bv = sizeof(float) * gemm::TV_PART * (size_t)parts;
  return max(b32, bv);
}

extern "C" int tmdnet_gemm_tn_f32_ws(int n_problems, const int* dims, const void* const* ptrs, void* workspace,
                                     size_t workspace_bytes, void* stream) {
  return gemm_tn(n_problems, dims, ptrs, 6, workspace, workspace_bytes, stream);
}

extern "C" int tmdnet_gemm_tn_rows_f32_ws(int n_problems, const int* dims, const void* const* ptrs, void* workspace,
                                          size_t workspace_bytes, void* stream) {
  return gemm_tn(n_problems, dims, ptrs, 7, workspace, workspace_bytes, stream);
}

extern "C" int tmdnet_proj_split_f32(int N, int K, const void* W, int ldw, void* Wp, void* stream) {
  if (N <= 0 || K <= 0 || !W || !Wp) return kBadArgument;
  if (K % 4 || ldw < K || ldw % 4 || (((uintptr_t)W) & 15) || (((uintptr_t)Wp) & 7)) return kUnsupported;
  const int n4 = N * K / 4;
  hipLaunchKernelGGL(proj::k_proj_split, dim3((n4 + 255) / 256), dim3(256), 0, (hipStream_t)stream, N, K,
                     (const float*)W, ldw, (unsigned short*)Wp);
  return hipGetLastError() == hipSuccess ? kOk : kLaunchFailed;
}

extern "C" int tmdnet_proj_f32(int M, int N, int K, const void* A, int lda, const void* Wp,
                               long long piece_stride, const void* bias, void* C, int ldc, void* stream) {
  if (M < 0 || N <= 0 || K <= 0 || !A || !Wp || !C) return kBadArgument;
  if (M == 0) return kOk;
  if ((K != 32 && K != 64) || N % 16 || lda < K || ldc < N || lda % 4 || ldc % 4 || piece_stride < (long long)N * K)
    return kUnsupported;
  if ((((uintptr_t)A) | ((uintptr_t)Wp) | ((uintptr_t)C) | ((uintptr_t)bias)) & 15) return kUnsupported;
  static const int mb_env = getenv("TMDNET_PROJ_MB") ? atoi(getenv("TMDNET_PROJ_MB")) : 0;
  static const int bn_env = getenv("TMDNET_PROJ_BN") ? atoi(getenv("TMDNET_PROJ_BN")) : 0;
  const bool big = M >= 65536;
  const int mb_req = mb_env ? mb_env : (big ? 4 : 2), bn_req = bn_env ? bn_env : (big ? 128 : 64);
  const int bn = (K == 64 && bn_req >= 128) ? 128 : 64;
  const int mb = mb_req >= 4 ? 4 : (mb_req >= 2 || bn == 128 || K == 32) ? 2 : 1;
  proj::Args P{M, N, lda, ldc, piece_stride, (const float*)A, (const unsigned short*)Wp, (const float*)bias,
               (float*)C};
  const dim3 g((N + bn - 1) / bn, (M + 64 * mb - 1) / (64 * mb));
  hipStream_t st = (hipStream_t)stream;
#define TMD_PROJ(KS_, MB_, BN_) hipLaunchKernelGGL((proj::k_proj_x3<KS_, MB_, BN_>), g, dim3(256), 0, st, P)
  if (K == 64) {
    if (bn == 128) {
      if (mb == 4) TMD_PROJ(2, 4, 128); else TMD_PROJ(2, 2, 128);
    } else {
      if (mb == 4) TMD_PROJ(2, 4, 64); else if (mb == 2) TMD_PROJ(2, 2, 64); else TMD_PROJ(2, 1, 64);
    }
  } else {
    if (mb == 4) TMD_PROJ(1, 4, 64); else TMD_PROJ(1, 2, 64);
  }
#undef TMD_PROJ
  return hipGetLastError() == hipSuccess ? kOk : kLaunchFailed;
}

extern "C" int tmdnet_split_t_f32(int N, int K, const void* B, int ldb, void* Bp, void* stream) {
  if (N <= 0 || K <= 0 || !B || !Bp) return kBadArgument;
  if (K % 4 || ldb < N || (((uintptr_t)Bp) & 7)) return kUnsupported;
  const int n = N * (K / 4);
  hipLaunchKernelGGL(proj::k_split_t, dim3((n + 255) / 256), dim3(256), 0, (hipStream_t)stream, N, K,
                     (const float*)B, ldb, (unsigned short*)Bp);
  return hipGetLastError() == hipSuccess ? kOk : kLaunchFailed;
}

extern "C" int tmdnet_gemm_x3_f32(int M, int N, int K, const void* A, int lda, const void* Bp, const void* bias,
                                  void* C, int ldc, int beta, void* stream) {
  return tmdnet_gemm_x3_ex_f32(M, N, K, A, lda, Bp, bias, C, ldc, beta, 0, nullptr, nullptr, nullptr, 0, stream);
}

static int gemm_x3_launch(int M, int N, int K, const void* A, int lda, const void* Bp, const void* W, int ldw, int ws,
                          const void* bias, void* C, int ldc, int beta, int act, void* pre, const void* rscale,
                          const void* dpre, int ldx, void* stream);

extern "C" int tmdnet_gemm_x3_ex_f32(int M, int N, int K, const void* A, int lda, const void* Bp, const void* bias,
                                     void* C, int ldc, int beta, int act, void* pre, const void* rscale,
                                     const void* dpre, int ldx, void* stream) {
  if (!Bp) return kBadArgument;
  return gemm_x3_launch(M, N, K, A, lda, Bp, nullptr, 0, 0, bias, C, ldc, beta, act, pre, rscale, dpre, ldx, stream);
}

extern "C" int tmdnet_gemm_x3w_f32(int M, int N, int K, const void* A, int lda, const void* W, int ldw, int trans_w,
                                   const void* bias, void* C, int ldc, int beta, int act, void* pre,
                                   const void* rscale, const void* dpre, int ldx, void* stream) {
  if (!W) return kBadArgument;
  if (ldw % 4 || (((uintptr_t)W) & 15) || ldw < (trans_w ? K : N)) return kUnsupported;
  return gemm_x3_launch(M, N, K, A, lda, nullptr, W, ldw, trans_w ? 1 : 2, bias, C, ldc, beta, act, pre, rscale,
                        dpre, ldx, stream);
}

static int gemm_x3_launch(int M, int N, int K, const void* A, int lda, const void* Bp, const void* W, int ldw, int ws,
                          const void* bias, void* C, int ldc, int beta, int act, void* pre, const void* rscale,
                          const void* dpre, int ldx, void* stream) {
  if (M < 0 || N <= 0 || K <= 0 || !A || !C) return kBadArgument;
  if (M == 0) return kOk;
  if (K % 32 || N % 16 || lda < K || ldc < N || lda % 4 || ldc % 4) return kUnsupported;
  if ((((uintptr_t)A) | ((uintptr_t)Bp) | ((uintptr_t)C) | ((uintptr_t)bias)) & 15) return kUnsupported;
  if ((pre || dpre) && (ldx < N || ldx % 4 || ((((uintptr_t)pre) | ((uintptr_t)dpre)) & 15))) return kUnsupported;
  static const int remap_env = [] {
    const char* e = getenv("TMDNET_X3_REMAP");
    return e ? atoi(e) : 1;
  }();
  proj::XArgs P{M, N, K, lda, ldc, beta ? 1 : 0, 0, 0, 0, (const float*)A, (const unsigned short*)Bp,
                (const float*)bias, (float*)C, act ? 1 : 0, ldx, (float*)pre, (const float*)rscale,
                (const float*)dpre, (const float*)W, ldw};
  hipStream_t st = (hipStream_t)stream;
  static const int bn_env = [] {
    const char* e = getenv("TMDNET_X3_BN");
    return e ? atoi(e) : 0;
  }();
  const int bn = bn_env == 64 || bn_env == 128 ? bn_env
                                               : (N <= 64 ? 64 : (N < 256 || M >= 131072) ? 128 : 64);
  P.nx = (N + bn - 1) / bn;
  P.ny = (M + 127) / 128;
  P.remap = remap_env && P.nx > 1 && (long long)P.nx * P.ny < (1ll << 31);
  const dim3 g = P.remap ? dim3(P.nx * P.ny) : dim3(P.nx, P.ny);
#define TMD_X3(WS_)                                                               \
  if (bn == 64)                                                                   \
    hipLaunchKernelGGL((proj::k_gemm_x3<2, 64, 1, WS_>), g, dim3(256), 0, st, P);  \
  else                                                                            \
    hipLaunchKernelGGL((proj::k_gemm_x3<2, 128, 4, WS_>), g, dim3(256), 0, st, P);
  if (ws == 1) {
    TMD_X3(1)
  } else if (ws == 2) {
    TMD_X3(2)
  } else {
    TMD_X3(0)
  }
#undef TMD_X3
  return hipGetLastError() == hipSuccess ? kOk : kLaunchFailed;
}
```

torchmd-net_amd/torchmdnet/_native.py:

```python
import ctypes
import os

import torch

_LIB_PATH = os.path.join(os.path.dirname(os.path.abspath(__file__)), "lib",
                         "libtmdnet_hip_debug.so" if os.environ.get("TMDNET_LIB") == "debug" else "libtmdnet_hip.so")

F32, F64 = 0, 1
NL_BRUTE, NL_SHARED, NL_CELL = 0, 1, 2
RBF_EXPNORM, RBF_GAUSS = 0, 1
ACC_VEC_RESIDUAL, ACC_EDGE = 1, 2
ACC_GRADS = 32
ET_V_PLANAR = 4
BWD2_ACC_EDGE, BWD2_ACC_GVEC = 8, 16
ET_TWO_PASS = 64

_STATUS = {1: "bad argument", 2: "unsupported configuration", 3: "kernel launch failed",
           4: "workspace too small"}

P = ctypes.c_void_p
I = ctypes.c_int
D = ctypes.c_double
SZ = ctypes.c_size_t

SIGNATURES = {
    "tmdnet_nl_workspace_bytes": (SZ, [I, I, P, D]),
    "tmdnet_nl_build": (I, [I, I, P, P, I, P, I, D, D, I, I, I, P, P, P, P, P, P, I, P, SZ, P]),
    "tmdnet_nl_build_paired": (I, [I, I, P, P, I, P, I, D, D, I, I, I, P, P, P, P, P, P, I, P, SZ, P, P, I, P]),
    "tmdnet_nl_backward": (I, [I, I, P, P, I, P, P, P, P, P, P]),
    "tmdnet_nl_backward_multi": (I, [I, I, P, P, I, P, P, P, P, P, P, P]),
    "tmdnet_nl_backward2": (I, [I, I, P, P, P, I, P, P, P, P, P, P, P, P]),
    "tmdnet_nl_backward_edges": (I, [I, I, P, I, P, P, P, P, P, P]),
    "tmdnet_edge_geom_fwd": (I, [I, I, I, I, P, P, P, P, P, P, D, D, P, P, P, P]),
    "tmdnet_edge_geom_fwd_rows": (I, [I, I, I, I, P, P, P, P, P, P, D, D, P, P, P, P, I, P, P]),
    "tmdnet_edge_geom_fwd_rows2": (I, [I, I, I, I, P, P, P, P, P, P, D, D, P, P, P, P, I, P, P, P]),
    "tmdnet_edge_geom_bwd": (I, [I, I, I, I, P, P, P, P, P, P, D, D, P, P, P, P, P, P]),
    "tmdnet_edge_geom_bwd_multi": (I, [I, I, I, I, P, P, P, P, P, P, D, D, P, P, P, P, P, P, P, P, P, P]),
    "tmdnet_edge_geom_bwd2": (I, [I, I, I, I, P, P, P, P, P, P, D, D, P, P, P, P, P, P, P, P, P, P, P]),
    "tmdnet_et_message_fwd": (I, [I, I, I, I, P, P, I, P, I, P, I, P, I, P, P, I, P, I, P, P, P, P, I, P, P,
                                  P]),
    "tmdnet_et_message_bwd": (I, [I, I, I, I, P, P, I, P, I, P, I, P, I, P, P, I, P, I, P, P, P, P,
                                  P, P, P, P, P, P, P, P, P, P, P, I, P, P, P]),
    "tmdnet_rbf_deriv": (I, [I, I, I, P, P, P, D, D, P, I, P, P]),
    "tmdnet_pair_index_workspace_bytes": (SZ, [I]),
    "tmdnet_pair_index": (I, [I, P, P, P, P, I, P, I, P, P, I, P, SZ, P]),
    "tmdnet_et_message_bwd2": (I, [I, I, I, I, P, P, I, P, I, P, I, P, I, P, P, I, P, I, P, P, P, P,
                                   P, P, P, P, P, I, P, I, P, P, P, P, P, P, P, P, P, P, P, P, I, P]),
    "tmdnet_et_message_bwd2_ex": (I, [I, I, I, I, P, P, P, I, P, I, P, I, P, I, P, P, I, P, I, P, P, P, P,
                                      P, I, P, I, P, I, P, P, I, P, I, P, P,
                                      P, P, P, I, P, I, P, I, P, P, I, P, I, P, P, P, P, P, I, P]),
    "tmdnet_et_epilogue_fwd": (I, [I, I, I, P, P, P, P, P, P, P, P]),
    "tmdnet_et_epilogue_bwd": (I, [I, I, I, P, P, P, P, P, P, P]),
    "tmdnet_et_epilogue_bwd_acc": (I, [I, I, I, P, P, P, P, P, P, I, P]),
    "tmdnet_et_epilogue_ln_fwd": (I, [I, I, I, P, P, P, P, P, P, P, D, P, P, P, P, P, P]),
    "tmdnet_ln_bwd_epilogue": (I, [I, I, I, P, P, P, P, P, P, P, P, P, P, P, P, P]),
    "tmdnet_ln_bwd_epilogue_w": (I, [I, I, I, P, P, P, P, P, P, P, P, P, P, P, P, P, P, I, P]),
    "tmdnet_et_oproj_epilogue_f32": (I, [I, I] + [P] * 11),
    "tmdnet_et_ln_mix_f32": (I, [I, I, P, P, P, D, P, P, I, P, P, P, P, P, P, I, P, P]),
    "tmdnet_et_lnbwd_oproj_f32": (I, [I, I] + [P] * 15),
    "tmdnet_et_adjoint_epi_ln": (I, [I, I, I] + [P] * 21),
    "tmdnet_et_adjoint_epi_ln2": (I, [I, I, I] + [P] * 22),
    "tmdnet_eq_head_fwd": (I, [I, I, I, P, P, P, P, P, P, P]),
    "tmdnet_eq_head_bwd": (I, [I, I, I, P, P, P, P, P, P]),
    "tmdnet_eq_head_bwd_weights": (I, [I, I, I, P, P, P, P, P, P, P, P]),
    "tmdnet_eq_head_hvp": (I, [I, I, I, P, P, P, P, P, P, P, P, P, P, P]),
    "tmdnet_nbr_embed_fwd": (I, [I, I, I, P, P, I, P, I, P, I, P, P, I, P, P, P]),
    "tmdnet_nbr_embed_bwd": (I, [I, I, I, P, P, I, P, I, P, I, P, P, I, P, P, P, P]),
    "tmdnet_nbr_embed_bwd2": (I, [I, I, I, P, P, P, I, P, I, P, I, P, P, I, P, P, P, P, P, P, P, P]),
    "tmdnet_tn_embed_fwd": (I, [I, I, I, P, P, I, D, P, I, P, P, P, I, P, P, P, P]),
    "tmdnet_tn_embed_bwd": (I, [I, I, I, P, P, I, D, P, I, P, P, P, I, P, P, P, P, P, P, P, P, P]),
    "tmdnet_tn_embed_bwd2": (I, [I, I, I, P, P, I, D, P, I, P, P, P, I, P, P, P, P, P, P, P, P, P, P, P, P, P, P,
                                 P]),
    "tmdnet_tn_message_fwd": (I, [I, I, I, P, P, I, D, P, I, P, I, P, P, P]),
    "tmdnet_tn_message_bwd": (I, [I, I, I, P, P, I, D, P, I, P, I, P, P, P, P, P]),
    "tmdnet_tn_message_bwd_add": (I, [I, I, I, P, P, I, D, P, I, P, I, P, P, P, P, P, P]),
    "tmdnet_tn_message_fwd_pairs": (I, [I, I, I, P, P, I, D, P, I, P, P, I, P, P, P]),
    "tmdnet_tn_message_bwd_pairs": (I, [I, I, I, P, P, I, D, P, I, P, P, I, P, I, P, P, P, P, P, P]),
    "tmdnet_tn_node_fwd": (I, [I, I, I, I, P, P, P, P]),
    "tmdnet_tn_node_bwd": (I, [I, I, I, I, P, P, P, P, P, P, P]),
    "tmdnet_tn_node_bwd2": (I, [I, I, I, I, P, P, P, P, P, P, P, P, P]),
    "tmdnet_silu_fwd": (I, [I, I, I, P, I, P, P, P]),
    "tmdnet_silu_bwd": (I, [I, I, I, P, I, P, P, I, P, P, P]),
    "tmdnet_mlp2_up": (I, [I, I, I, P, I, P, P, I, P, P, P, P, P, P, P, P]),
    "tmdnet_mlp2_down": (I, [I, I, I, P, I, P, P, P, P]),
    "tmdnet_atom_sum_fwd": (I, [I, I, I, P, P, P, P, P, P]),
    "tmdnet_atom_sum_bwd": (I, [I, I, I, P, P, P, P, P]),
    "tmdnet_dot_sum_fwd": (I, [I, I, I, P, I, P, P, I, P, P, P, P, P]),
    "tmdnet_dot_sum_bwd": (I, [I, I, I, P, P, I, P, P, P, P]),
    "tmdnet_dot_sum_fwd_atoms": (I, [I, I, I, P, I, P, P, I, P, P, P, P, P, P]),
    "tmdnet_layernorm_fwd_f32": (I, [I, I, P, I, P, P, D, P, I, P, P, P]),
    "tmdnet_layernorm_bwd_f32": (I, [I, I, P, I, P, P, P, P, I, P, I, P]),
    "tmdnet_layernorm_bwd2_f32": (I, [I, I, P, I, P, P, P, P, I, P, P, P, P, P, P, P]),
    "tmdnet_layernorm_wgrad_workspace_bytes": (SZ, [I, I]),
    "tmdnet_layernorm_wgrad_f32": (I, [I, I, P, I, P, P, P, I, P, P, P, SZ, P]),
    "tmdnet_gemm_f32": (I, [I, P, P, P]),
    "tmdnet_gemm_ex_f32": (I, [I, P, P, P]),
    "tmdnet_gemm_tn_f32": (I, [I, P, P, P]),
    "tmdnet_gemm_tn_workspace_bytes": (ctypes.c_size_t, [I, P]),
    "tmdnet_gemm_tn_f32_ws": (I, [I, P, P, P, ctypes.c_size_t, P]),
    "tmdnet_gemm_tn_rows_f32_ws": (I, [I, P, P, P, ctypes.c_size_t, P]),
    "tmdnet_embedding_bwd_f32": (I, [I, I, I, P, I, P, P, P, I, P]),
    "tmdnet_embedding_fwd_f32": (I, [I, I, I, P, I, P, P, P, P, P]),
    "tmdnet_proj_split_f32": (I, [I, I, P, I, P, P]),
    "tmdnet_split_t_f32": (I, [I, I, P, I, P, P]),
    "tmdnet_gemm_x3_f32": (I, [I, I, I, P, I, P, P, P, I, I, P]),
    "tmdnet_gemm_x3_ex_f32": (I, [I, I, I, P, I, P, P, P, I, I, I, P, P, P, I, P]),
    "tmdnet_gemm_x3w_f32": (I, [I, I, I, P, I, P, I, I, P, P, I, I, I, P, P, P, I, P]),
    "tmdnet_fep_image_bytes": (SZ, [I, I]),
    "tmdnet_fep_split_f32": (I, [I, I, P, I, P, P, P, P, P]),
    "tmdnet_et_fused_bwd_f32": (I, [I, I, I, I, P, P, I, P, I, P, I, P, I, P, P, P, P, P, P, ctypes.c_longlong, P, P, P,
                                    P, P, P, P, P, P, P, P, P, I, P, SZ, P]),
    "tmdnet_et_fused_bwd_workspace_bytes": (SZ, [I]),
    "tmdnet_et_fused_fwd_f32": (I, [I, I, I, I, P, P, I, P, I, P, I, P, I, P, P, P, P, P, ctypes.c_longlong, P, P, P, P, P,
                                    I, P]),
    "tmdnet_nbr_fused_fwd_f32": (I, [I, I, I, P, P, I, P, I, P, P, P, ctypes.c_longlong, P, P, P, P, I, P, P, P]),
    "tmdnet_nbr_fused_bwd_f32": (I, [I, I, I, P, P, I, P, I, P, P, P, P, ctypes.c_longlong, P, P, P, P, I, P, P, I,
                                     P]),
    "tmdnet_eq_head_x3_f32": (I, [I, I, P, P, P, P, P, P, P, P, P]),
    "tmdnet_eq_head_x3_pieces_bytes": (SZ, [I]),
    "tmdnet_eq_head_x3_split_f32": (I, [I, P, P, P]),
    "tmdnet_fep_frags_bytes": (SZ, [ctypes.c_longlong, I]),
    "tmdnet_fep_frags_f32": (I, [ctypes.c_longlong, I, P, P, P, D, D, I, P, P, P]),
    "tmdnet_proj_f32": (I, [I, I, I, P, I, P, ctypes.c_longlong, P, P, I, P]),
    "tmdnet_mse2_fwd": (I, [I, I, P, P, D, I, P, P, D, P, P]),
    "tmdnet_mse2_bwd": (I, [I, I, P, P, D, I, P, P, D, P, P, P, P]),
    "tmdnet_build_info": (ctypes.c_char_p, []),
    "tmdnet_set_tuning": (I, [I, I]),
}

_lib = None
_torch_ops_loaded = False
_TORCH_OPS_PATH = os.path.join(os.path.dirname(os.path.abspath(__file__)), "lib", "libtmdnet_torch.so")


def load_torch_ops():
    global _torch_ops_loaded
    if _torch_ops_loaded:
        return
    if not os.path.exists(_TORCH_OPS_PATH):
        raise RuntimeError(f"torchmd-net_amd: operator library not found at {_TORCH_OPS_PATH}; run `make`")
    torch.ops.load_library(_TORCH_OPS_PATH)
    _torch_ops_loaded = True


def invalidate_stack_cache():
    if _torch_ops_loaded:
        torch.ops.tmdnet.et_stack_invalidate()


def library_path():
    return _LIB_PATH


def load(required=True):
    global _lib
    if _lib is not None:
        return _lib
    if not os.path.exists(_LIB_PATH):
        if required:
            raise RuntimeError(
                f"torchmd-net_amd: HIP library not found at {_LIB_PATH}; run `make` (or "
                "__graft_entry__.build()) -- there is no CPU fallback for the hot path")
        return None
    lib = ctypes.CDLL(_LIB_PATH)
    for name, (res, args) in SIGNATURES.items():
        fn = getattr(lib, name)
        fn.restype = res
        fn.argtypes = args
    _lib = lib
    return lib


def check(rc, what):
    if rc != 0:
        raise RuntimeError(f"torchmd-net_amd: {what} failed: {_STATUS.get(rc, rc)}")


def require_gpu(t, what):
    if not t.is_cuda:
        raise RuntimeError(
            f"torchmd-net_amd: {what} runs only on a ROCm GPU (got a {t.device} tensor); this "
            "package has no CPU implementation of the hot path")


def dtype_code(dtype):
    if dtype == torch.float32:
        return F32
    if dtype == torch.float64:
        return F64
    raise RuntimeError(f"torchmd-net_amd: unsupported floating type {dtype} (float32/float64)")


def ptr(t):
    return None if t is None else ctypes.c_void_p(t.data_ptr())


def stream(device=None):
    return ctypes.c_void_p(torch.cuda.current_stream(device).cuda_stream)
```

torchmd-net_amd/torchmdnet/et_stack.py:

```python
import contextlib
import os
import weakref

import torch
import torch.nn.functional as F
from torch.autograd import Function

from . import _native as nat
from . import kernels

_EPS = 1e-5


def _stack_views(params):
    buf = torch.cat([p.detach() for p in params], 0)
    off = 0
    for p in params:
        n = p.shape[0]
        p.data = buf[off:off + n]
        off += n
    return buf


def _is_stacked(buf, params):
    if buf is None:
        return False
    es = buf.element_size()
    row = buf[0].numel() if buf.dim() > 1 else 1
    off = 0
    for p in params:
        if p.device != buf.device or p.dtype != buf.dtype or not p.is_contiguous() \
                or p.data_ptr() != buf.data_ptr() + off * row * es:
            return False
        off += p.shape[0]
    return off == buf.shape[0]


class LayerWeights:

    def __init__(self, layer):
        self.layer = layer
        self.bufs = {}

    def _get(self, name, params):
        buf = self.bufs.get(name)
        if not _is_stacked(buf, params):
            buf = _stack_views(params)
            self.bufs[name] = buf
        return buf

    def fused(self):
        L = self.layer
        qkv_w = self._get("qkv_w", [L.q_proj.weight, L.k_proj.weight, L.v_proj.weight])
        qkv_b = self._get("qkv_b", [L.q_proj.bias, L.k_proj.bias, L.v_proj.bias])
        return qkv_w, qkv_b


class StackWeights:

    def __init__(self, layers):
        self.layers = layers
        self.bufs = {}

    def _get(self, name, params):
        buf = self.bufs.get(name)
        if not _is_stacked(buf, params):
            buf = _stack_views(params)
            self.bufs[name] = buf
        return buf

    def dkv(self):
        mods = [m for layer in self.layers for m in (layer.dk_proj, layer.dv_proj) if m is not None]
        if not mods:
            return None, None
        return self._get("w", [m.weight for m in mods]), self._get("b", [m.bias for m in mods])


BATCH_DKV_BYTES = 2 << 30
PLANAR_MIN_EDGES = 131072
PAIR_ROWS = True
FEP = os.environ.get("TMDNET_FEP", "auto")
FEP_MIN_EDGES = int(os.environ.get("TMDNET_FEP_MIN_EDGES", "131072"))
FEP_BWD = os.environ.get("TMDNET_FEP_BWD", "fused")
FUSED_BWD = FEP_BWD == "fused"
DR_MODE = os.environ.get("TMDNET_DR", "auto")
SECOND_ORDER = os.environ.get("TMDNET_ET_SECOND_ORDER", "hand")
RECORD_IN_FORCE_PASS = os.environ.get("TMDNET_ET_RECORD", "1") not in ("0", "off")
_EXPECT_SECOND_ORDER = [False]
PROJ_WGRAD = os.environ.get("TMDNET_PROJ_WGRAD", "tn")
NODE_WGRAD = os.environ.get("TMDNET_NODE_WGRAD", "tn")


@contextlib.contextmanager
def second_order_expected(on=True):
    prev = _EXPECT_SECOND_ORDER[0]
    _EXPECT_SECOND_ORDER[0] = bool(on)
    try:
        yield
    finally:
        _EXPECT_SECOND_ORDER[0] = prev

_PERMS = {}


def _v_perm(H, heads, device):
    key = ("v", H, heads, str(device))
    if key not in _PERMS:
        d = H // heads
        j = torch.arange(3 * H)
        part, rem = j // H, j % H
        _PERMS[key] = (rem // d * 3 * d + part * d + rem % d).to(device)
    return _PERMS[key]


def _planar_perms(meta, device):
    key = ("stack", meta.H, meta.heads, meta.n_layers, meta.hk, meta.hv, str(device))
    if key not in _PERMS:
        H = meta.H
        vp = _v_perm(H, meta.heads, device)
        qkv = torch.cat([torch.arange(2 * H, device=device), 2 * H + vp])
        per = ([torch.arange(H, device=device)] if meta.hk else []) + \
            ([H * int(meta.hk) + vp] if meta.hv else [])
        one = torch.cat(per) if per else torch.zeros(0, dtype=torch.long, device=device)
        dkv = torch.cat([l * meta.D + one for l in range(meta.n_layers)])
        inv = lambda p: torch.empty_like(p).scatter_(0, p, torch.arange(p.numel(), device=device))
        _PERMS[key] = (qkv, inv(qkv), dkv, inv(dkv), one, inv(one))
    return _PERMS[key]


def layer_params(layer):
    ps = [layer.layernorm.weight, layer.layernorm.bias, layer.q_proj.weight, layer.q_proj.bias,
          layer.k_proj.weight, layer.k_proj.bias, layer.v_proj.weight, layer.v_proj.bias,
          layer.vec_proj.weight, layer.o_proj.weight, layer.o_proj.bias]
    if layer.dk_proj is not None:
        ps += [layer.dk_proj.weight, layer.dk_proj.bias]
    if layer.dv_proj is not None:
        ps += [layer.dv_proj.weight, layer.dv_proj.bias]
    return ps


class _Meta:

    def __init__(self, graph, heads, H, hk, hv, n_layers, fused, acc_nodes=None, dkv_w=None, dkv_b=None,
                 batched=False):
        self.graph = graph
        self.heads = heads
        self.H = H
        self.hk = hk
        self.hv = hv
        self.n_layers = n_layers
        self.fused = fused
        self.D = (int(hk) + 3 * int(hv)) * H
        self.dkv_w, self.dkv_b = dkv_w, dkv_b
        self.batched = batched
        self.planar = False
        self.flags = 0
        self.acts = 0
        self.qkv_eff = fused
        self.dkv_eff = (dkv_w, dkv_b)
        self.np = 11 + 2 * int(hk) + 2 * int(hv)
        self.pairs = None
        self.pk_rows = None
        self.rbf = None
        self.out_norm = False
        self.f_pairs = None
        self.fdp_pairs = None
        self.dkv_wp = None
        self.fep = False
        self.fep_imgs = None
        self.grad_mode = True

    def split(self, params):
        return [params[i * self.np:(i + 1) * self.np] for i in range(self.n_layers)]

    def dkv_split(self):
        if self.dkv_wp is None and self.dkv_eff[0] is not None:
            self.dkv_wp = kernels.proj_split(self.dkv_eff[0])
        return self.dkv_wp

    def dkv_proj(self, A, l=None, bias=True):
        w, b = self.dkv_eff if l is None else self.dkv_layer(l)
        return kernels.proj(A, w, b if bias else None, wp=self.dkv_split(), row0=0 if l is None else l * self.D)

    def dkv_layer(self, l):
        w, b_ = self.dkv_eff
        if w is None:
            return None, None
        a, b = l * self.D, (l + 1) * self.D
        return w[a:b], b_[a:b]

    def refresh_effective(self):
        self.dkv_wp = None
        if not self.planar:
            self.qkv_eff, self.dkv_eff = self.fused, (self.dkv_w, self.dkv_b)
            return
        qp, _, dp, _, _, _ = self.perms
        self.qkv_eff = [(w.index_select(0, qp), b.index_select(0, qp)) for w, b in self.fused]
        self.dkv_eff = (self.dkv_w.index_select(0, dp), self.dkv_b.index_select(0, dp)) \
            if self.dkv_w is not None else (None, None)


def _epilogue_fwd(x, vec, vecp, o, veca):
    lib = nat.load()
    N, H = x.shape
    xo = torch.empty_like(x)
    vo = torch.empty_like(veca)
    rc = lib.tmdnet_et_epilogue_fwd(nat.dtype_code(x.dtype), N, H, nat.ptr(x), nat.ptr(vec),
                                    nat.ptr(vecp), nat.ptr(o), nat.ptr(veca), nat.ptr(xo), nat.ptr(vo),
                                    nat.stream(x.device))
    nat.check(rc, "tmdnet_et_epilogue_fwd")
    return xo, vo


def _epilogue_bwd(gx, gvec, vecp, o, g_vecp, g_o, acc=False):
    lib = nat.load()
    N, H = gx.shape
    rc = lib.tmdnet_et_epilogue_bwd_acc(nat.dtype_code(gx.dtype), N, H, nat.ptr(gx), nat.ptr(gvec),
                                        nat.ptr(vecp), nat.ptr(o), nat.ptr(g_vecp), nat.ptr(g_o), int(acc),
                                        nat.stream(gx.device))
    nat.check(rc, "tmdnet_et_epilogue_bwd_acc")


def _epi_ln(x, vec, vecp, o, veca, ln_w, ln_b, xn_out=None, vo_out=None):
    lib = nat.load()
    N, H = x.shape
    xo = torch.empty_like(x) if o is not None else None
    vo = (vo_out if vo_out is not None else torch.empty_like(veca)) if o is not None else None
    xn = xn_out if xn_out is not None else torch.empty_like(x)
    mean = torch.empty((N, 1), dtype=x.dtype, device=x.device)
    rstd = torch.empty((N, 1), dtype=x.dtype, device=x.device)
    rc = lib.tmdnet_et_epilogue_ln_fwd(nat.dtype_code(x.dtype), N, H, nat.ptr(x), nat.ptr(vec), nat.ptr(vecp),
                                       nat.ptr(o), nat.ptr(veca), nat.ptr(ln_w), nat.ptr(ln_b), _EPS,
                                       nat.ptr(xo), nat.ptr(vo), nat.ptr(xn), nat.ptr(mean), nat.ptr(rstd),
                                       nat.stream(x.device))
    nat.check(rc, "tmdnet_et_epilogue_ln_fwd")
    return xo, vo, xn, mean, rstd


NODE_FUSE = os.environ.get("TMDNET_ET_NODE_FUSE", "1") != "0"


def _node_fuse_ok(x):
    N, H = x.shape
    return (NODE_FUSE and x.is_cuda and x.dtype == torch.float32 and H % 64 == 0 and H <= 256
            and 3 * N <= kernels.GEMM_MAX_ROWS)


def _ln_mix(x, ln_w, ln_b, w, b, vec, vec_w, xn_out):
    lib = nat.load()
    N, H = x.shape
    qkv = torch.empty((N, w.shape[0]), dtype=x.dtype, device=x.device)
    mean = torch.empty((N, 1), dtype=x.dtype, device=x.device)
    rstd = torch.empty((N, 1), dtype=x.dtype, device=x.device)
    vecp = torch.empty((N, 3, vec_w.shape[0]), dtype=x.dtype, device=x.device) if vec is not None else None
    w, ln_w, ln_b = w.contiguous(), ln_w.contiguous(), ln_b.contiguous()
    vec_w = vec_w.contiguous() if vec is not None else None
    rc = lib.tmdnet_et_ln_mix_f32(N, H, nat.ptr(x), nat.ptr(ln_w), nat.ptr(ln_b), _EPS, nat.ptr(w), nat.ptr(b),
                                  w.shape[0], nat.ptr(qkv), nat.ptr(xn_out), nat.ptr(mean), nat.ptr(rstd),
                                  nat.ptr(vec), nat.ptr(vec_w), vec_w.shape[0] if vec is not None else 0,
                                  nat.ptr(vecp), nat.stream(x.device))
    nat.check(rc, "tmdnet_et_ln_mix_f32")
    return qkv, vecp, xn_out, mean, rstd


def _oproj_epi(xa, o_w, o_b, x, vec, vecp, veca, vo_out):
    lib = nat.load()
    N, H = x.shape
    o = torch.empty((N, o_w.shape[0]), dtype=x.dtype, device=x.device)
    xo = torch.empty_like(x)
    o_w = o_w.contiguous()
    rc = lib.tmdnet_et_oproj_epilogue_f32(N, H, nat.ptr(xa), nat.ptr(o_w), nat.ptr(o_b), nat.ptr(x), nat.ptr(vec),
                                          nat.ptr(vecp), nat.ptr(veca), nat.ptr(o), nat.ptr(xo), nat.ptr(vo_out),
                                          nat.stream(x.device))
    nat.check(rc, "tmdnet_et_oproj_epilogue_f32")
    return o, xo, vo_out


def _ln_bwd_oproj(g_xn, x, mean, rstd, ln_w, g_res, g_vec, vecp, o, o_w, g_vecp, g_o):
    lib = nat.load()
    N, H = x.shape
    gx = torch.empty_like(x)
    gxa = torch.empty_like(x)
    rc = lib.tmdnet_et_lnbwd_oproj_f32(N, H, nat.ptr(g_xn), nat.ptr(x), nat.ptr(mean), nat.ptr(rstd), nat.ptr(ln_w),
                                       nat.ptr(g_res), nat.ptr(g_vec), nat.ptr(vecp), nat.ptr(o), nat.ptr(o_w),
                                       nat.ptr(gx), nat.ptr(g_vecp), nat.ptr(g_o), nat.ptr(gxa), nat.stream(x.device))
    nat.check(rc, "tmdnet_et_lnbwd_oproj_f32")
    return gx, gxa


def _ln_bwd_epi(g_xn, x, mean, rstd, ln_w, g_res, g_vec, vecp, o, g_vecp, g_o, wrows=None, g_res2=None, acc=False):
    lib = nat.load()
    N, H = x.shape
    g_x = torch.empty_like(g_xn)
    rc = lib.tmdnet_ln_bwd_epilogue_w(nat.dtype_code(x.dtype), N, H, nat.ptr(g_xn), nat.ptr(x), nat.ptr(mean),
                                      nat.ptr(rstd), nat.ptr(ln_w), nat.ptr(g_res), nat.ptr(g_res2), nat.ptr(g_x),
                                      nat.ptr(g_vec), nat.ptr(vecp), nat.ptr(o), nat.ptr(g_vecp), nat.ptr(g_o),
                                      nat.ptr(wrows), int(acc), nat.stream(x.device))
    nat.check(rc, "tmdnet_ln_bwd_epilogue_w")
    return g_x


def _pair_f(meta, f):
    if meta.pairs is None:
        return f
    return meta.f_pairs if meta.f_pairs is not None else f.index_select(0, meta.pairs[1])


def _act_pkv(meta, acts, l, f):
    a = acts[l]
    if a[7] is None and meta.fep_imgs is not None and meta.D:
        if meta.batched:
            pkv_all, D = meta.dkv_proj(_pair_f(meta, f)), meta.D
            for j in range(meta.n_layers):
                acts[j] = acts[j][:7] + (pkv_all[:, j * D:(j + 1) * D],) + acts[j][8:]
        else:
            acts[l] = a[:7] + (meta.dkv_proj(_pair_f(meta, f), l),) + a[8:]
    return acts[l]


def _forward_layers(meta, x, f, C, u, params, r=None, want_bwd=False):
    H = meta.H
    N = x.shape[0]
    vec = None
    acts = []
    D = meta.D
    meta.refresh_effective()
    fep = meta.fep and r is not None and (not want_bwd or (FEP_BWD != "off" and not _EXPECT_SECOND_ORDER[0]))
    if not fep:
        meta.fep_imgs = None
    fp = _pair_f(meta, f) if (D and not fep) else f
    pkv_all = meta.dkv_proj(fp) if (meta.batched and D and not fep) else None
    layers = meta.split(params)
    L = len(layers)
    od = dict(dtype=x.dtype, device=x.device)
    xn_all, xa_all = torch.empty((L, N, H), **od), torch.empty((L, N, H), **od)
    vec_all = torch.empty((L, N, 3, H), **od)
    meta.stk = (xn_all, xa_all, vec_all)
    nf = _node_fuse_ok(x)
    if not nf:
        _, _, xn, mean, rstd = _epi_ln(x, None, None, None, None, layers[0][0], layers[0][1], xn_out=xn_all[0])
    for l, p in enumerate(layers):
        vec_w, o_w, o_b = p[8], p[9], p[10]
        qkv_w, qkv_b = meta.qkv_eff[l]
        dkv_w, dkv_b = meta.dkv_layer(l)
        if nf:
            qkv, vecp, xn, mean, rstd = _ln_mix(x, p[0], p[1], qkv_w, qkv_b, vec, vec_w, xn_all[l])
        else:
            qkv = torch.empty((N, qkv_w.shape[0]), dtype=x.dtype, device=x.device)
            probs = [(xn, qkv_w, True, qkv_b, qkv, False)]
            vecp = None
            if vec is not None:
                vecp = torch.empty((N, 3, 3 * H), dtype=x.dtype, device=x.device)
                probs.append((vec.view(3 * N, H), vec_w, True, None, vecp.view(3 * N, 3 * H), False))
            kernels.gemm_group(probs)
        xa = xa_all[l]
        veca = torch.empty((N, 3, H), dtype=x.dtype, device=x.device)
        if fep:
            pkv = None
            if l == 0:
                meta.fep_imgs = []
                meta.fep_frag = kernels.fep_frag_shared(meta.graph, r, meta.rbf)
            if not meta.planar:
                one = _planar_perms(meta, x.device)[4]
                dkv_w, dkv_b = dkv_w.index_select(0, one), dkv_b.index_select(0, one)
            meta.fep_imgs.append(kernels.fep_split(dkv_w, dkv_b))
            kernels.et_fused_fwd_launch(qkv[:, :H], qkv[:, H:2 * H], qkv[:, 2 * H:], vec, C, u,
                                        meta.fep_imgs[l], meta.fep_frag, meta.graph, meta.heads, xa, veca,
                                        flags=meta.flags)
        else:
            if pkv_all is not None:
                pkv = pkv_all[:, l * D:(l + 1) * D]
            else:
                pkv = meta.dkv_proj(fp, l) if dkv_w is not None else None
            pk = pkv[:, :H] if meta.hk else None
            pv = pkv[:, H * int(meta.hk):] if meta.hv else None
            kernels.et_message_fwd_launch(qkv[:, :H], qkv[:, H:2 * H], qkv[:, 2 * H:], vec, pk, pv, C, u,
                                          meta.graph, meta.heads, xa, veca, meta.flags, meta.pk_rows)
        if nf and l + 1 < len(layers):
            o, x_next, vec_next = _oproj_epi(xa, o_w, o_b, x, vec, vecp, veca, vec_all[l + 1])
            acts.append((x, vec, xn, mean, rstd, qkv, vecp, pkv, xa, o))
            x, vec = x_next, vec_next
            continue
        o = torch.empty((N, o_w.shape[0]), dtype=x.dtype, device=x.device)
        kernels.gemm_group([(xa, o_w, True, o_b, o, False)])
        acts.append((x, vec, xn, mean, rstd, qkv, vecp, pkv, xa, o))
        if l + 1 < len(layers):
            x, vec, xn, mean, rstd = _epi_ln(x, vec, vecp, o, veca, layers[l + 1][0], layers[l + 1][1],
                                             xn_out=xn_all[l + 1], vo_out=vec_all[l + 1])
        elif meta.out_norm:
            x_pre, vec, x, mean, rstd = _epi_ln(x, vec, vecp, o, veca, params[-2], params[-1])
            acts.append((x_pre, mean, rstd))
        else:
            x, vec = _epilogue_fwd(x, vec, vecp, o, veca)
    return x, vec, acts


def _backward_layers(meta, gX, gV, f, C, u, params, acts, need_ws, r=None, dr=False, record=None, inject=None,
                     seed_pre_norm=False, want_f=True):
    H = meta.H
    N = gX.shape[0]
    graph = meta.graph
    E = graph.n_edges
    o = dict(dtype=gX.dtype, device=gX.device)
    has_e = meta.hk or meta.hv
    D = meta.D
    rec = record is not None
    inj = inject or {}
    stk = inj.get("stk")
    acc = stk is not None

    def injected(key, l):
        lst = inj.get(key)
        return None if lst is None else lst[l]

    zbuf = torch.empty(((5 if dr else 4) * E,), **o)
    g_C, g_u = zbuf[:E], zbuf[E:4 * E].view(E, 3)
    g_r = None
    fused = (dr and meta.fep and not rec and not inj and meta.fep_imgs is not None and FUSED_BWD
             and all(a[7] is None for a in acts[:meta.n_layers]))
    if dr:
        assert has_e and not any(need_ws) and meta.rbf is not None
        g_r = zbuf[4 * E:]
        if not fused:
            if meta.fdp_pairs is not None and meta.pairs is not None:
                fdp = meta.fdp_pairs
            else:
                fdp = kernels.rbf_deriv(r, *meta.rbf, rows=meta.pairs[1] if meta.pairs is not None else None)
            dpkv_all = meta.dkv_proj(fdp, bias=False) if meta.batched else None
    if has_e and (not dr or rec):
        if acc and stk.get("pkv") is not None and (meta.batched or rec):
            g_pkv_all = stk["pkv"]
        else:
            g_pkv_all = torch.empty((E, meta.n_layers * D if (meta.batched or rec) else D), **o)
    g_f = None
    new = lambda shape: torch.empty(shape, **o)
    L = meta.n_layers
    if acc:
        g_qkv_all, g_o_all, g_vecp_all = stk["qkv"], stk["o"], stk["vecp"]
    else:
        g_qkv_all, g_o_all, g_vecp_all = new((L, N, 5 * H)), new((L, N, 3 * H)), new((L, N, 3, 3 * H))
    g_xn_all = new((L, N, H))
    any_w = any(need_ws[:L])
    ln_rows = new((L, N, H)) if any_w else None
    gvec_bufs = [new((N, 3, H)), new((N, 3, H))]
    layers = meta.split(params)
    g_params = [None] * len(params)
    epi_done = False
    bwd_nf = (not acc and not inj and not any(need_ws[:meta.n_layers + 1]) and gX is not None and H == 128
              and _node_fuse_ok(gX))
    g_xa_pre = None
    x_top = inj.get("x_top")
    if meta.out_norm and not seed_pre_norm:
        x_pre, mean_o, rstd_o = acts[meta.n_layers]
        last = acts[meta.n_layers - 1]
        if need_ws[meta.n_layers]:
            g_y = gX
            gX = _ln_bwd_epi(g_y, x_pre, mean_o, rstd_o, params[-2], x_top, None, None, None, None, None)
            g_params[-2:] = list(kernels.layer_norm_wgrad(g_y, x_pre, mean_o, rstd_o))
        elif x_top is not None:
            gX = _ln_bwd_epi(gX, x_pre, mean_o, rstd_o, params[-2], x_top, None, None, None, None, None)
        elif bwd_nf and gV is not None:
            gX, g_xa_pre = _ln_bwd_oproj(gX, x_pre, mean_o, rstd_o, params[-2], None, gV, last[6], last[9],
                                         layers[L - 1][9], g_vecp_all[L - 1], g_o_all[L - 1])
            epi_done = True
        else:
            gX = _ln_bwd_epi(gX, x_pre, mean_o, rstd_o, params[-2], None, gV, last[6], last[9], g_vecp_all[L - 1],
                             g_o_all[L - 1])
            epi_done = True
    elif x_top is not None:
        gX = gX + x_top
    for l in reversed(range(meta.n_layers)):
        p = layers[l]
        x, vec, xn, mean, rstd, qkv, vecp, pkv, xa, o_ = acts[l] if fused else _act_pkv(meta, acts, l, f)
        ln_w, ln_b = p[0], p[1]
        vec_w, o_w = p[8], p[9]
        qkv_w, _ = meta.qkv_eff[l]
        dkv_w, _ = meta.dkv_layer(l)
        g_qkv, g_o, g_vecp = g_qkv_all[l], g_o_all[l], g_vecp_all[l]
        gpk = gpv = dpk = dpv = None
        if dr and not fused:
            dpkv = dpkv_all[:, l * D:(l + 1) * D] if meta.batched else meta.dkv_proj(fdp, l, bias=False)
            dpk = dpkv[:, :H] if meta.hk else None
            dpv = dpkv[:, H * int(meta.hk):] if meta.hv else None
        if has_e and (not dr or rec):
            g_pkv = g_pkv_all[:, l * D:(l + 1) * D] if (meta.batched or rec) else g_pkv_all
            if acc and not (meta.batched or rec):
                g_pkv.copy_(stk["pkv"][:, l * D:(l + 1) * D])
            gpk = g_pkv[:, :H] if meta.hk else None
            gpv = g_pkv[:, H * int(meta.hk):] if meta.hv else None
        if rec:
            step = {"gX": gX, "gV": gV}
        if not epi_done:
            _epilogue_bwd(gX, gV, vecp, o_, g_vecp, g_o, acc=acc)
        if not acc and injected("o", l) is not None:
            g_o.add_(injected("o", l))
            if vecp is not None:
                g_vecp.add_(injected("vecp", l))
        if g_xa_pre is not None:
            g_xa, g_xa_pre = g_xa_pre, None
        else:
            g_xa = torch.empty((N, H), **o)
            kernels.gemm_group([(g_o, o_w, False, None, g_xa, False)])
        g_vec_in = gvec_bufs[l % 2] if vec is not None else None
        if acc and vec is not None:
            g_vec_in = injected("vec", l) if injected("vec", l) is not None else torch.zeros((N, 3, H), **o)
        flags = (nat.ACC_VEC_RESIDUAL | (nat.ACC_EDGE if l < L - 1 else 0) | meta.flags
                 | (nat.ACC_GRADS if acc else 0))
        if fused:
            kernels.et_fused_bwd_launch(qkv[:, :H], qkv[:, H:2 * H], qkv[:, 2 * H:], vec, C, u, meta.fep_imgs[l],
                                        meta.fep_frag, graph, meta.heads, g_xa, gV, g_qkv[:, :H], g_qkv[:, H:2 * H],
                                        g_qkv[:, 2 * H:], g_vec_in, g_C, g_u, g_r, accumulate=flags)
        else:
            pk = pkv[:, :H] if meta.hk else None
            pv = pkv[:, H * int(meta.hk):] if meta.hv else None
            kernels.et_message_bwd_launch(
                qkv[:, :H], qkv[:, H:2 * H], qkv[:, 2 * H:], vec, pk, pv, C, u, graph, meta.heads, g_xa, gV,
                g_qkv[:, :H], g_qkv[:, H:2 * H], g_qkv[:, 2 * H:], g_vec_in, gpk, gpv, g_C, g_u,
                accumulate=flags, pk_rows=meta.pk_rows, dpk=dpk, dpv=dpv, g_r=g_r)
        if not acc:
            if injected("qkv", l) is not None:
                g_qkv.add_(injected("qkv", l))
            if has_e and not dr and injected("pkv", l) is not None:
                g_pkv.add_(injected("pkv", l))
            if g_vec_in is not None and injected("vec", l) is not None:
                g_vec_in.add_(injected("vec", l))
        if has_e and not (meta.batched or rec) and not dr:
            if not want_f:
                pass
            elif g_f is None:
                g_f = torch.mm(g_pkv, dkv_w)
            else:
                g_f.addmm_(g_pkv, dkv_w)
        g_xn = g_xn_all[l]
        probs = [(g_qkv, qkv_w, False, None, g_xn, False)]
        if vec is not None:
            probs.append((g_vecp.view(3 * N, 3 * H), vec_w, False, None, g_vec_in.view(3 * N, H), True))
        kernels.gemm_group(probs)
        if rec:
            step.update(g_o=g_o, g_vecp=g_vecp if vec is not None else None, g_xa=g_xa, g_qkv=g_qkv, g_xn=g_xn)
            record.append(step)
            gvec_bufs = [new((N, 3, H)), new((N, 3, H))]
        need_w = need_ws[l]
        prev = acts[l - 1] if l > 0 else None
        if bwd_nf and prev is not None:
            g_x, g_xa_pre = _ln_bwd_oproj(g_xn, x, mean, rstd, ln_w, gX, g_vec_in, prev[6], prev[9], layers[l - 1][9],
                                          g_vecp_all[l - 1], g_o_all[l - 1])
        else:
            g_x = _ln_bwd_epi(g_xn, x, mean, rstd, ln_w, gX, g_vec_in,
                              prev[6] if prev else None, prev[9] if prev else None,
                              g_vecp_all[l - 1] if prev else None, g_o_all[l - 1] if prev else None,
                              wrows=ln_rows[l] if any_w else None, g_res2=injected("x", l), acc=acc)
        epi_done = prev is not None
        if need_w and has_e and not (meta.batched or rec):
            base = l * meta.np
            g_w, g_b = torch.mm(g_pkv.t(), f), g_pkv.sum(0)
            if meta.planar:
                oinv = meta.perms[5]
                g_w, g_b = g_w.index_select(0, oinv), g_b.index_select(0, oinv)
            gl = _dkv_param_grads(meta, g_w, g_b)
            g_params[base + 11:base + 11 + len(gl)] = gl
        gX = g_x
        gV = g_vec_in
    adj = inj.get("W")
    if any_w:
        _node_weight_grads(meta, g_params, need_ws, g_qkv_all, g_o_all, g_vecp_all, g_xn_all, ln_rows, adj)
    if rec:
        record.append({"g_pkv": g_pkv_all if has_e else None, "stacks": (g_qkv_all, g_o_all, g_vecp_all),
                       "dpkv": dpkv_all if dr else None})
    if has_e and (meta.batched or rec) and not dr:
        g_f = torch.mm(g_pkv_all, meta.dkv_eff[0]) if want_f else None
        if any(need_ws[:meta.n_layers]):
            if PROJ_WGRAD == "tn":
                g_w_all, g_b_all = kernels._linear_wgrad(g_pkv_all, f, True, True,
                                                         seg2=adj.get("dkv") if adj is not None else None,
                                                         rows=_edge_rows(meta.graph, g_pkv_all))
            else:
                g_w_all = torch.mm(g_pkv_all.t(), f)
                if adj is not None and adj.get("dkv") is not None:
                    g_w_all.addmm_(adj["dkv"][0].t(), adj["dkv"][1])
                g_b_all = g_pkv_all.sum(0)
            if meta.planar:
                dinv = meta.perms[3]
                g_w_all, g_b_all = g_w_all.index_select(0, dinv), g_b_all.index_select(0, dinv)
            for l in range(meta.n_layers):
                if need_ws[l]:
                    base = l * meta.np + 11
                    a, b = l * D, (l + 1) * D
                    gl = _dkv_param_grads(meta, g_w_all[a:b], g_b_all[a:b])
                    g_params[base:base + len(gl)] = gl
    return gX, g_f, g_C, g_u, g_r, g_params
# ... 373 lines not shown
        out.append(any(want_params[-2:]))
    return out


def _dkv_param_grads(meta, g_w, g_b):
    H = meta.H
    out = []
    if meta.hk:
        out += [g_w[:H], g_b[:H]]
    if meta.hv:
        a = H * int(meta.hk)
        out += [g_w[a:], g_b[a:]]
    return out


def composite_stack(meta, x, f, C, u, params, message=None):
    H = meta.H
    graph = meta.graph
    src, dst = graph.src.long(), graph.dst.long()
    N = x.shape[0]
    vec = torch.zeros((N, 3, H), dtype=x.dtype, device=x.device)
    layers = meta.split(params)
    D = meta.D
    pkv_layers = None
    if D:
        rest = [p[11:] for p in layers]
        w_all = torch.cat([w for r in rest for w in r[0::2]], 0)
        b_all = torch.cat([b for r in rest for b in r[1::2]], 0)
        pkv_layers = torch.split(F.linear(f, w_all, b_all), D, dim=1)
    for l, p in enumerate(layers):
        ln_w, ln_b, q_w, q_b, k_w, k_b, v_w, v_b, vec_w, o_w, o_b = p[:11]
        xn = F.layer_norm(x, (H,), ln_w, ln_b, _EPS)
        q, k, v = torch.split(F.linear(xn, torch.cat((q_w, k_w, v_w)), torch.cat((q_b, k_b, v_b))),
                              [q_w.shape[0], k_w.shape[0], v_w.shape[0]], dim=1)
        vec1, vec2, vec3 = torch.split(F.linear(vec, vec_w), H, dim=-1)
        vec_dot = (vec1 * vec2).sum(dim=1)
        pk = pv = None
        if D:
            hk_w = H * int(meta.hk)
            pk, pv = torch.split(pkv_layers[l], [hk_w, D - hk_w], dim=1)
            pk = pk if meta.hk else None
            pv = pv if meta.hv else None
        if message is None:
            xa, veca = kernels.et_message_composite(q, k, v, vec, pk, pv, C, u, src, dst, N, meta.heads, meta.acts)
        else:
            xa, veca = message(q, k, v, vec, pk, pv, C, u)
        o1, o2, o3 = torch.split(F.linear(xa, o_w, o_b), H, dim=1)
        x = x + vec_dot * o2 + o3
        vec = vec + vec3 * o1.unsqueeze(1) + veca
    if meta.out_norm:
        x = F.layer_norm(x, (H,), params[-2], params[-1], _EPS)
    return x, vec


_HANDED_OFF = []


def check_pending_consumed():
    left = [m for m in (ref() for ref in _HANDED_OFF) if m is not None and getattr(m, "pending", None) is not None]
    _HANDED_OFF.clear()
    for m in left:
        m.pending = None
    if kernels.head_pending_left():
        raise RuntimeError("torchmd-net_amd: the output head's second-order weight terms were not consumed by "
                           "the head's backward (engine order); the parameter gradients are incomplete")
    if left:
        raise RuntimeError("torchmd-net_amd: the ET stack's second-order cotangents were not consumed by the "
                           "forward node's backward (engine order); the parameter gradients are incomplete")


def _will_run(node):
    if node is None:
        return False
    try:
        return bool(torch._C._will_engine_execute_node(node))
    except RuntimeError:
        return True


class _ETStack(Function):
    @staticmethod
    def forward(ctx, meta, x, f, C, u, r, *params):
        want = meta.grad_mode and any(ctx.needs_input_grad)
        x_out, vec_out, acts = _forward_layers(meta, x, f, C, u, params, r=r, want_bwd=want)
        ctx.meta = meta
        ctx.acts = acts
        meta.fwd_node = weakref.ref(ctx)
        meta.pending = None
        ctx.save_for_backward(x, f, C, u, r, *params)
        return x_out, vec_out

    @staticmethod
    def backward(ctx, gX, gV):
        x, f, C, u, r, *params = ctx.saved_tensors
        meta = ctx.meta
        nf = ctx.next_functions
        off = len(nf) - len(params)
        need_w = tuple(any(_will_run(nf[off + l * meta.np + j][0]) for j in range(meta.np))
                       for l in range(meta.n_layers))
        if meta.out_norm:
            base = off + meta.n_layers * meta.np
            need_w += (_will_run(nf[base][0]) or _will_run(nf[base + 1][0]),)
        if gX is None:
            gX = torch.zeros_like(x)
        if gV is None:
            gV = torch.zeros((x.shape[0], 3, meta.H), dtype=x.dtype, device=x.device)
        pending, meta.pending = getattr(meta, "pending", None), None
        dr = bool(meta.rbf is not None and ctx.needs_input_grad[5] and meta.D and not any(need_w))
        if DR_MODE in ("0", "off") or pending is not None:
            dr = False
        want_f = f is not None and ctx.needs_input_grad[2] and _will_run(nf[1][0])
        if pending is not None:
            ti = [i for i, t in zip(range(2, 7), (f, C, u, r)) if t is not None]
            idx = {i: 1 + j for j, i in enumerate(ti)}
            pending["want_cu"] = any(ctx.needs_input_grad[i] and _will_run(nf[idx[i]][0]) for i in (3, 4)
                                     if i in idx)
        record = (dr and torch.is_grad_enabled() and _EXPECT_SECOND_ORDER[0] and SECOND_ORDER != "composite"
                  and RECORD_IN_FORCE_PASS and hand_second_order_ok(meta, dr, need_w, ()))
        outs = _ETStackBwd.apply(meta, ctx.acts, need_w, dr, pending, want_f, record, gX.contiguous(),
                                 gV.contiguous(), x, f, C, u, r, *params)
        g_x, g_f, g_C, g_u, g_r = outs[:5]
        return (None, g_x, g_f, g_C, g_u, g_r) + tuple(outs[5:])


class _ETStackBwd(Function):
    @staticmethod
    def forward(ctx, meta, acts, need_w, dr, pending, want_f, record, gX, gV, x, f, C, u, r, *params):
        if not meta.graph.symmetric:
            raise RuntimeError("torchmd-net_amd: the ET backward source pass needs a symmetric edge "
                               "list (include_transpose=True, no capacity overflow)")
        ctx.rec = None
        if record:
            rec = []
            g_x, g_f, g_C, g_u, g_r, g_params = _backward_layers(meta, gX, gV, f, C, u, params, acts, need_w,
                                                                 r=r, dr=True, record=rec, want_f=False)
            ctx.rec, ctx.g_f0 = rec, None
        else:
            g_x, g_f, g_C, g_u, g_r, g_params = _backward_layers(meta, gX, gV, f, C, u, params, acts, need_w,
                                                                 r=r, dr=dr,
                                                                 inject=pending["inj"] if pending else None,
                                                                 want_f=want_f)
        if pending is not None:
            if pending.get("want_cu", True):
                g_C = g_C + pending["C_bar"]
                g_u = g_u + pending["u_bar"]
            else:
                g_C = g_u = None
            wl = list(need_w)
            g_params = _apply_w_bar(meta, list(g_params), pending["W_bar"], pending["on_bar"],
                                    lambda i: wl[min(i // meta.np, len(wl) - 1)] if i < meta.n_layers * meta.np
                                    else wl[-1])
        ctx.meta = meta
        ctx.dr = dr
        ctx.acts = acts
        ctx.need_w = need_w
        ctx.save_for_backward(gX, gV, x, f, C, u, r, *params)
        return (g_x, g_f, g_C, g_u, g_r) + tuple(g_params)

    @staticmethod
    def backward(ctx, *ggs):
        saved = ctx.saved_tensors
        meta = ctx.meta
        graph, heads = meta.graph, meta.heads

        def message(q, k, v, vec, pk, pv, C_, u_):
            return kernels.et_message(q, k, v, vec, pk, pv, C_, u_, graph, heads, meta.acts)
# ... 92 lines not shown
```

torchmd-net_amd/torchmdnet/kernels.py:

```python
import ctypes
import math
import os
import weakref
from collections import namedtuple

import torch
import torch.nn.functional as F
from torch.autograd import Function

from . import _native as nat

HEAD_SECOND_ORDER = os.environ.get("TMDNET_HEAD_SECOND_ORDER", "hand")
HEAD_HANDOFF = os.environ.get("TMDNET_HEAD_HANDOFF", "1") == "1"
_HEAD_HANDED = []


class _HeadLink:
    __slots__ = ("fwd", "hvp", "pending", "__weakref__")

    def __init__(self, fwd, hvp):
        self.fwd, self.hvp, self.pending = fwd, hvp, None

    def other_will_run(self, side):
        node = (self.hvp if side == "fwd" else self.fwd)()
# ... 1321 lines not shown
        rc = lib.tmdnet_gemm_x3w_f32(M, N, K, A.data_ptr(), A.stride(0), B.data_ptr(), B.stride(0), int(bool(tb)),
                                     nat.ptr(bias), C.data_ptr(), C.stride(0), *epi, st)
        if rc != GEMM_UNSUPPORTED:
            nat.check(rc, "tmdnet_gemm_x3w_f32")
            return True
    bp = torch.empty((3, N, K), dtype=torch.int16, device=A.device)
    split = lib.tmdnet_proj_split_f32 if tb else lib.tmdnet_split_t_f32
    rc = split(N, K, B.data_ptr(), B.stride(0), bp.data_ptr(), st)
    if rc == GEMM_UNSUPPORTED:
        return False
    nat.check(rc, "tmdnet_split")
    rc = lib.tmdnet_gemm_x3_ex_f32(M, N, K, A.data_ptr(), A.stride(0), bp.data_ptr(), nat.ptr(bias), C.data_ptr(),
                                   C.stride(0), *epi, st)
    if rc == GEMM_UNSUPPORTED:
        return False
    nat.check(rc, "tmdnet_gemm_x3_ex_f32")
    return True


def gemm_lib(p):
    Bop = p.B.t() if p.trans_b else p.B
    if p.beta:
        p.C.addmm_(p.A, Bop)
        if p.bias is not None:
            p.C.add_(p.bias)
    elif p.bias is not None:
        torch.addmm(p.bias, p.A, Bop, out=p.C)
    else:
        torch.mm(p.A, Bop, out=p.C)
    return p.C


def gemm_group(problems):
    ps = [Gemm(*p) for p in problems]
    if gemm_launch(ps):
        return
    for p in ps:
        if p.A.shape[0] > GEMM_MAX_ROWS:
            if gemm_x3(*p[:6]):
                continue
        elif len(ps) > 1 and gemm_launch([p]):
            continue
        gemm_lib(p)


def gemm_ex_launch(p):
    p = Gemm(*p)
    return gemm_x3(*p) if p.A.shape[0] > GEMM_MAX_ROWS else gemm_launch([p])


PROJ = os.environ.get("TMDNET_PROJ", "x3")


def proj_split(W):
    N, K = W.shape
    if not (PROJ == "x3" and W.is_cuda and W.dtype == torch.float32 and W.stride(1) == 1 and K in (32, 64)
            and N % 16 == 0):
        return None
    wp = torch.empty((3, N, K), dtype=torch.int16, device=W.device)
    rc = nat.load().tmdnet_proj_split_f32(N, K, W.data_ptr(), W.stride(0), wp.data_ptr(), nat.stream(W.device))
    if rc == GEMM_UNSUPPORTED:
        return None
    nat.check(rc, "tmdnet_proj_split_f32")
    return wp


def proj(A, W, bias=None, out=None, wp=None, row0=0):
    M, K = A.shape
    N = W.shape[0]
    if out is None:
        out = torch.empty((M, N), dtype=A.dtype, device=A.device)
    if (PROJ == "x3" and A.is_cuda and A.dtype == torch.float32 and A.stride(1) == 1 and out.stride(1) == 1
            and (bias is None or bias.is_contiguous())):
        if wp is None:
            wp, row0 = proj_split(W), 0
        if wp is not None:
            rc = nat.load().tmdnet_proj_f32(M, N, K, A.data_ptr(), A.stride(0), wp[0, row0:].data_ptr(),
                                            wp.shape[1] * K, None if bias is None else bias.data_ptr(),
                                            out.data_ptr(), out.stride(0), nat.stream(A.device))
            if rc != GEMM_UNSUPPORTED:
                nat.check(rc, "tmdnet_proj_f32")
                return out
    return gemm_lib(Gemm(A, W, True, bias, out, False))


def wgrad_tn(problems):
    if not problems:
        return
    fp32 = all(p["A"].dtype == torch.float32 and p["A"].is_cuda for p in problems)
    if fp32:
        for i in range(0, len(problems), 32):
            _wgrad_tn_launch(problems[i:i + 32])
        return
    for p in problems:
        C, Cb = p["C"], p.get("Cb")
        ncol = C.shape[1] + int(Cb is not None)
        res = None
        for A, B, ones in ((p["A"], p.get("B"), p.get("ones", False)), (p.get("A2"), p.get("B2"), p.get("ones2", False))):
            if A is None or A.shape[0] == 0:
                continue
            Bx = B
            if ones:
                one = torch.ones((A.shape[0], 1), dtype=A.dtype, device=A.device)
                Bx = one if B is None else torch.cat((B, one), 1)
            elif B is not None and B.shape[1] < ncol:
                Bx = torch.cat((B, torch.zeros((A.shape[0], 1), dtype=A.dtype, device=A.device)), 1)
            t = A.t() @ Bx
            res = t if res is None else res + t
        outs = [(C, res)] if Cb is None else [(C, res[:, :-1]), (Cb, res[:, -1])]
        for dst, val in outs:
            if p.get("beta"):
                dst.add_(val)
            else:
                dst.copy_(val)


def _wgrad_tn_launch(problems):
    lib = nat.load()
    n = len(problems)
    dims = (ctypes.c_int * (12 * n))()
    npp = 7 if any(p.get("rows") is not None for p in problems) else 6
    ptrs = (ctypes.c_void_p * (npp * n))()
    keep = []
    for i, p in enumerate(problems):
        A, B, C, Cb = p["A"], p.get("B"), p["C"], p.get("Cb")
        A2, B2 = p.get("A2"), p.get("B2")
        for t in (A, B, A2, B2, C, Cb):
            if t is not None and t.stride(-1) != 1:
                raise RuntimeError("wgrad_tn: operands need unit column stride")
        keep += [A, B, A2, B2, C, Cb]
        K2 = 0 if A2 is None else A2.shape[0]
        N = C.shape[1] + int(Cb is not None) if C.dim() == 2 else 1
        dims[12 * i:12 * i + 12] = [A.shape[1], N, A.shape[0], K2, A.stride(0),
                                    0 if B is None else B.stride(0), 0 if A2 is None else A2.stride(0),
                                    0 if B2 is None else B2.stride(0), C.stride(0) if C.dim() == 2 else 1,
                                    int(bool(p.get("beta"))), int(bool(p.get("ones"))), int(bool(p.get("ones2")))]
        rows = p.get("rows")
        if rows is not None and (rows.dtype != torch.int32 or rows.numel() != 1 or rows.device != A.device):
            raise RuntimeError("wgrad_tn: rows must be an int32 device scalar")
        ts = (A, B, A2, B2, C, Cb) + ((rows,) if npp == 7 else ())
        ptrs[npp * i:npp * i + npp] = [None if t is None else t.data_ptr() for t in ts]
    dev = problems[0]["A"].device
    wsb = lib.tmdnet_gemm_tn_workspace_bytes(n, dims)
    ws = torch.empty((max(wsb, 4) // 4,), dtype=torch.float32, device=dev) if wsb else None
    fn = lib.tmdnet_gemm_tn_rows_f32_ws if npp == 7 else lib.tmdnet_gemm_tn_f32_ws
    rc = fn(n, dims, ptrs, None if ws is None else ws.data_ptr(), wsb, nat.stream(dev))
    nat.check(rc, "tmdnet_gemm_tn_f32_ws")


ATOM_SUM_MAX_MOLECULES = 8192


def _atom_sum_composite(x, batch, n_mol, std, mean):
    out = torch.zeros((n_mol,) + tuple(x.shape[1:]), dtype=x.dtype, device=x.device).index_add(0, batch, x * std)
    return out + mean


class _AtomSum(Function):

    @staticmethod
    def forward(ctx, x, batch, n_mol, std, mean):
        lib = nat.load()
        y = torch.empty((n_mol, 1), dtype=x.dtype, device=x.device)
        rc = lib.tmdnet_atom_sum_fwd(nat.dtype_code(x.dtype), x.shape[0], n_mol, nat.ptr(x), nat.ptr(batch),
                                     nat.ptr(std), nat.ptr(mean), nat.ptr(y), nat.stream(x.device))
        nat.check(rc, "tmdnet_atom_sum_fwd")
# ... 1248 lines not shown
```

Baseline: 37840 molecules/s.

## Fuse distance-projection activation and derivative into projection GEMM epilogue

Adds a projection kernel that applies the key/value filter activation in its epilogue. It also computes the chain-ruled derivative rows (activation derivative times the projected RBF derivative) in the same pass. The ET message forward and force-pass backward kernels gain a PRE mode that consumes these pre-activated rows directly and skips per-edge activation evaluation and derivative recomputation. The path is enabled by default but restricted to batched, non-FEP, fp32 and first-order cases. The cost is extra stored derivative buffers and more memory traffic from writing both S and D for every layer.

After: 39260 molecules/s, median of 6. 3.7% higher.

```diff
diff --git a/include/tmdnet.h b/include/tmdnet.h
--- a/include/tmdnet.h
+++ b/include/tmdnet.h
@@ -17,6 +17,7 @@
 enum { TMDNET_ET_V_PLANAR = 4 };
 enum { TMDNET_BWD2_ACC_EDGE = 8, TMDNET_BWD2_ACC_GVEC = 16 };
 enum { TMDNET_ET_TWO_PASS = 64 };
+enum { TMDNET_ET_PREACT = 128 };
 enum { TMDNET_ACT_SILU = 0, TMDNET_ACT_SSP = 1, TMDNET_ACT_TANH = 2, TMDNET_ACT_SIGMOID = 3 };
 #define TMDNET_ET_ACT(kv, attn) (((kv) << 8) | ((attn) << 12))
 
@@ -333,6 +334,9 @@
 int tmdnet_proj_split_f32(int N, int K, const void* W, int ldw, void* Wp, void* stream);
 int tmdnet_proj_f32(int M, int N, int K, const void* A, int lda, const void* Wp, long long piece_stride,
                     const void* bias, void* C, int ldc, void* stream);
+int tmdnet_proj_act_f32(int M, int N, int K, const void* A, const void* dA, int lda, const void* Wp,
+                        long long piece_stride, const void* bias, int act, void* S, void* D, int ldc,
+                        void* stream);
 
 size_t tmdnet_fep_image_bytes(int D, int R);
 int tmdnet_fep_split_f32(int D, int R, const void* W, int ldw, const void* bias, void* img, void* wsc,
diff --git a/torchmd-net_amd/csrc/et_message.hip b/torchmd-net_amd/csrc/et_message.hip
--- a/torchmd-net_amd/csrc/et_message.hip
+++ b/torchmd-net_amd/csrc/et_message.hip
@@ -126,6 +126,11 @@
     }
   }
 }
+template <typename T, int V>
+__device__ __forceinline__ void preact(const T (&x)[V], bool has, T (&s)[V]) {
+#pragma unroll
+  for (int i = 0; i < V; ++i) s[i] = has ? x[i] : T(1);
+}
 template <typename T> __device__ __forceinline__ const T* opt(const T* p, size_t off, const T* dummy) {
   return p ? p + off : dummy;
 }
@@ -250,7 +255,7 @@
   }
 }
 
-template <typename T, int V, int S, int CS, bool ORD, bool GA = true>
+template <typename T, int V, int S, int CS, bool ORD, bool GA = true, bool PRE = false>
 __global__ __launch_bounds__(256) void k_fwd(Args<T> A) {
   const int AKV = GA ? A.act_kv : kActSilu, AAT = GA ? A.act_at : kActSilu;
   __shared__ T lds[S > 1 ? 4 * 64 * 4 * V : 1];
@@ -293,11 +298,20 @@
       ldv<T, V>(w2, vecs + 2 * vcd);
       pre();
       if (!hw) { zero(w0); zero(w1); zero(w2); }
-      T dk[V], dvx[V], dv1[V], dv2[V], dd[V];
-      act<T, V>(st.k, hk, dk, dd, AKV);
-      act<T, V>(st.x, hv, dvx, dd, AKV);
-      act<T, V>(st.a, hv, dv1, dd, AKV);
-      act<T, V>(st.b, hv, dv2, dd, AKV);
+      T dk[V], dvx[V], dv1[V], dv2[V];
+      if constexpr (PRE) {
+        (void)AKV;
+        preact<T, V>(st.k, hk, dk);
+        preact<T, V>(st.x, hv, dvx);
+        preact<T, V>(st.a, hv, dv1);
+        preact<T, V>(st.b, hv, dv2);
+      } else {
+        T dd[V];
+        act<T, V>(st.k, hk, dk, dd, AKV);
+        act<T, V>(st.x, hv, dvx, dd, AKV);
+        act<T, V>(st.a, hv, dv1, dd, AKV);
+        act<T, V>(st.b, hv, dv2, dd, AKV);
+      }
       T part = T(0);
 #pragma unroll
       for (int i = 0; i < V; ++i) part += q[i] * kk[i] * dk[i];
@@ -354,8 +368,9 @@
     for (long long i = tid; i < rows; i += nth) A.gr[e0 + i] = T(0);
 }
 
-template <typename T, int V, int S, int CS, bool DR, bool AG = false, bool GA = true>
+template <typename T, int V, int S, int CS, bool DR, bool AG = false, bool GA = true, bool PRE = false>
 __device__ __forceinline__ void bwd_dst_body(const Args<T>& A, int blk, int nwg) {
+  static_assert(!PRE || (DR && !AG), "pre-activated rows: the dr-mode force pass only");
   const int AKV = GA ? A.act_kv : kActSilu, AAT = GA ? A.act_at : kActSilu;
   __shared__ T lds[S > 1 ? 4 * 64 * V : 1];
   const Geo G = geo<S, CS, false>(A.n, A.L, nullptr, A.xcd, blk, nwg);
@@ -434,11 +449,20 @@
       const T (&px)[V] = st.x;
       const T (&p1)[V] = st.a;
       const T (&p2)[V] = st.b;
-      T dk[V], ddk[V], dvx[V], dv1[V], dv2[V], ddx[V], dd1[V], dd2[V];
-      act<T, V>(pk, hk, dk, ddk, AKV);
-      act<T, V>(px, hv, dvx, ddx, AKV);
-      act<T, V>(p1, hv, dv1, dd1, AKV);
-      act<T, V>(p2, hv, dv2, dd2, AKV);
+      constexpr int VD = PRE ? 1 : V;
+      T dk[V], ddk[VD], dvx[V], dv1[V], dv2[V], ddx[VD], dd1[VD], dd2[VD];
+      if constexpr (PRE) {
+        (void)AKV;
+        preact<T, V>(pk, hk, dk);
+        preact<T, V>(px, hv, dvx);
+        preact<T, V>(p1, hv, dv1);
+        preact<T, V>(p2, hv, dv2);
+      } else {
+        act<T, V>(pk, hk, dk, ddk, AKV);
+        act<T, V>(px, hv, dvx, ddx, AKV);
+        act<T, V>(p1, hv, dv1, dd1, AKV);
+        act<T, V>(p2, hv, dv2, dd2, AKV);
+      }
       T part = T(0), ga = T(0), gu0 = T(0), gu1 = T(0), gu2 = T(0);
 #pragma unroll
       for (int i = 0; i < V; ++i) {
@@ -458,12 +482,21 @@
 #pragma unroll
       for (int i = 0; i < V; ++i) {
         gq[i] += gs * kk[i] * dk[i];
-        gpk[i] = gs * q[i] * kk[i] * ddk[i];
-        gpx[i] = gx[i] * a * vx[i] * ddx[i];
-        const T gv1e = g0[i] * w0[i] + g1[i] * w1[i] + g2[i] * w2[i];
-        gp1[i] = gv1e * v1[i] * dd1[i];
-        const T gv2e = g0[i] * u0 + g1[i] * u1 + g2[i] * u2;
-        gp2[i] = gv2e * v2[i] * dd2[i];
+        if constexpr (PRE) {
+          gpk[i] = gs * q[i] * kk[i];
+          gpx[i] = gx[i] * a * vx[i];
+          const T gv1e = g0[i] * w0[i] + g1[i] * w1[i] + g2[i] * w2[i];
+          gp1[i] = gv1e * v1[i];
+          const T gv2e = g0[i] * u0 + g1[i] * u1 + g2[i] * u2;
+          gp2[i] = gv2e * v2[i];
+        } else {
+          gpk[i] = gs * q[i] * kk[i] * ddk[i];
+          gpx[i] = gx[i] * a * vx[i] * ddx[i];
+          const T gv1e = g0[i] * w0[i] + g1[i] * w1[i] + g2[i] * w2[i];
+          gp1[i] = gv1e * v1[i] * dd1[i];
+          const T gv2e = g0[i] * u0 + g1[i] * u1 + g2[i] * u2;
+          gp2[i] = gv2e * v2[i] * dd2[i];
+        }
       }
       const T gc = group_sum(head_leader ? ga * sa.s : T(0), A.L);
       gu0 = group_sum(gu0, A.L);
@@ -476,7 +509,7 @@
           grr += (hk ? gpk[i] * dpk_[i] : T(0)) +
                  (hv ? gpx[i] * dpx_[i] + gp1[i] * dp1_[i] + gp2[i] * dp2_[i] : T(0));
         grr = group_sum(grr, A.L);
-        if (on && (A.gpk || A.gpv)) {
+        if (!PRE && on && (A.gpk || A.gpv)) {
           if (hk && A.gpk) stv<T, V>(A.gpk + (size_t)k * A.ldpk + c0, gpk);
           if (hv && A.gpv) {
             T* gp = A.gpv + (size_t)k * A.ldpv + vo;
@@ -518,7 +551,7 @@
   zero_pad_rows(A, blk, nwg);
 }
 
-template <typename T, int V, int S, int CS, bool GA = true>
+template <typename T, int V, int S, int CS, bool GA = true, bool PRE = false>
 __device__ __forceinline__ void bwd_src_body(const Args<T>& A, int blk, int nwg) {
   const int AKV = GA ? A.act_kv : kActSilu, AAT = GA ? A.act_at : kActSilu;
   __shared__ T lds[S > 1 ? 4 * 64 * 7 * V : 1];
@@ -574,11 +607,20 @@
       const T (&px)[V] = st.x;
       const T (&p1)[V] = st.a;
       const T (&p2)[V] = st.b;
-      T dk[V], ddk[V], dvx[V], dv1[V], dv2[V], dd[V];
-      act<T, V>(pk, hk, dk, ddk, AKV);
-      act<T, V>(px, hv, dvx, dd, AKV);
-      act<T, V>(p1, hv, dv1, dd, AKV);
-      act<T, V>(p2, hv, dv2, dd, AKV);
+      T dk[V], dvx[V], dv1[V], dv2[V];
+      if constexpr (PRE) {
+        (void)AKV;
+        preact<T, V>(pk, hk, dk);
+        preact<T, V>(px, hv, dvx);
+        preact<T, V>(p1, hv, dv1);
+        preact<T, V>(p2, hv, dv2);
+      } else {
+        T ddk[V], dd[V];
+        act<T, V>(pk, hk, dk, ddk, AKV);
+        act<T, V>(px, hv, dvx, dd, AKV);
+        act<T, V>(p1, hv, dv1, dd, AKV);
+        act<T, V>(p2, hv, dv2, dd, AKV);
+      }
       T part = T(0), ga = T(0);
 #pragma unroll
       for (int i = 0; i < V; ++i) {
@@ -647,19 +689,19 @@
 template <typename T, int V, bool DR>
 constexpr int bwd_min_waves() { return (DR && sizeof(T) == 4 && V <= 4) ? 3 : 1; }
 
-template <typename T, int V, int S, int CS, bool DR, bool AG = false, bool GA = true>
+template <typename T, int V, int S, int CS, bool DR, bool AG = false, bool GA = true, bool PRE = false>
 __global__ __launch_bounds__(256, (bwd_min_waves<T, V, DR>())) void k_bwd_dst(Args<T> A) {
-  bwd_dst_body<T, V, S, CS, DR, AG, GA>(A, blockIdx.x, gridDim.x);
-}
-template <typename T, int V, int S, int CS, bool GA = true>
+  bwd_dst_body<T, V, S, CS, DR, AG, GA, PRE>(A, blockIdx.x, gridDim.x);
+}
+template <typename T, int V, int S, int CS, bool GA = true, bool PRE = false>
 __global__ __launch_bounds__(256) void k_bwd_src(Args<T> A) {
-  bwd_src_body<T, V, S, CS, GA>(A, blockIdx.x, gridDim.x);
-}
-template <typename T, int V, int S, int CS, bool DR, bool AG = false, bool GA = true>
+  bwd_src_body<T, V, S, CS, GA, PRE>(A, blockIdx.x, gridDim.x);
+}
+template <typename T, int V, int S, int CS, bool DR, bool AG = false, bool GA = true, bool PRE = false>
 __global__ __launch_bounds__(256, (bwd_min_waves<T, V, DR>())) void k_bwd_both(Args<T> A) {
   const int split = (int)gridDim.x / 2;
-  if ((int)blockIdx.x < split) bwd_dst_body<T, V, S, CS, DR, AG, GA>(A, blockIdx.x, split);
-  else bwd_src_body<T, V, S, CS, GA>(A, blockIdx.x - split, split);
+  if ((int)blockIdx.x < split) bwd_dst_body<T, V, S, CS, DR, AG, GA, PRE>(A, blockIdx.x, split);
+  else bwd_src_body<T, V, S, CS, GA, PRE>(A, blockIdx.x - split, split);
 }
 
 template <typename T, int V, int S, int PD, bool GA = true>
@@ -1434,7 +1476,7 @@
 template <typename T, int V, int S, int KIND, bool ORD>
 static int et_launch_vs(Args<T> A, hipStream_t st) {
   int cs = 1;
-  if (KIND == 1 || A.H % (cs * V) || (A.H / cs / V) & (A.H / cs / V - 1) || A.H / cs / V < A.lph ||
+  if (KIND == 1 || KIND == 11 || A.H % (cs * V) || (A.H / cs / V) & (A.H / cs / V - 1) || A.H / cs / V < A.lph ||
       A.H / cs / V > 64)
     cs = 1;
   A.HC = A.H / cs;
@@ -1456,6 +1498,10 @@
   else if (KIND == 4) hipLaunchKernelGGL((k_bwd_dst<T, V, S, 1, true, false, GA>), g, b, 0, st, A);
   else if (KIND == 5) hipLaunchKernelGGL((k_bwd_both<T, V, S, 1, true, false, GA>), dim3(2 * nbn), b, 0, st, A);
   else if (KIND == 6) hipLaunchKernelGGL((k_bwd_both<T, V, S, 1, false, true, GA>), dim3(2 * nbn), b, 0, st, A);
+  else if (KIND == 10) hipLaunchKernelGGL((k_fwd<T, V, S, 1, ORD, GA, true>), g, b, 0, st, A);
+  else if (KIND == 11) hipLaunchKernelGGL((k_bwd_dst<T, V, S, 1, true, false, GA, true>), g, b, 0, st, A);
+  else if (KIND == 12) hipLaunchKernelGGL((k_bwd_src<T, V, S, 1, GA, true>), g, b, 0, st, A);
+  else if (KIND == 13) hipLaunchKernelGGL((k_bwd_both<T, V, S, 1, true, false, GA, true>), dim3(2 * nbn), b, 0, st, A);
   else if (KIND == 8 || KIND == 9) {
     const size_t node = (size_t)(4 / S) * 12 * A.H, red = S > 1 ? 4 * 64 * 8 * V : 1;
     const size_t bytes = (node > red ? node : red) * sizeof(T);
@@ -1482,9 +1528,10 @@
 static int et_launch_v(const Args<T>& A, hipStream_t st) {
   int S = et_waves_per_node(A.n, (int)sizeof(T) * V);
   static const bool env_s_set = getenv("TMDNET_ET_S") != nullptr;
-  if (KIND == 0 && !env_s_set && (int)sizeof(T) * V <= 32) S = 4;
+  constexpr bool FWD = KIND == 0 || KIND == 10;
+  if (FWD && !env_s_set && (int)sizeof(T) * V <= 32) S = 4;
   static const int bwd_s = getenv("TMDNET_ET_BWD_S") ? atoi(getenv("TMDNET_ET_BWD_S")) : 0;
-  if (KIND != 0 && bwd_s && (int)sizeof(T) * V <= 32) S = bwd_s >= 4 ? 4 : bwd_s >= 2 ? 2 : 1;
+  if (!FWD && bwd_s && (int)sizeof(T) * V <= 32) S = bwd_s >= 4 ? 4 : bwd_s >= 2 ? 2 : 1;
   if (S == 4) return et_launch_vs<T, V, (sizeof(T) * V <= 32 ? 4 : 1), KIND, ORD>(A, st);
   if (S == 2) return et_launch_vs<T, V, (sizeof(T) * V <= 32 ? 2 : 1), KIND, ORD>(A, st);
   return et_launch_vs<T, V, 1, KIND, ORD>(A, st);
@@ -1561,6 +1608,7 @@
   if (flags & TMDNET_ET_V_PLANAR) { A.planar = 1; A.vst = H; }
   A.xo = (T*)xo;
   A.veco = (T*)veco;
+  if (flags & TMDNET_ET_PREACT) return order ? et_launch<T, 10, true>(V, A, st) : et_launch<T, 10, false>(V, A, st);
   return order ? et_launch<T, 0, true>(V, A, st) : et_launch<T, 0, false>(V, A, st);
 }
 
@@ -1593,6 +1641,12 @@
   if (dr && ((A.pk && !dpk) || (A.pv && !dpv))) return kBadArgument;
   if (!dr && ((A.pk && !gpk) || (A.pv && !gpv))) return kBadArgument;
   const int fuse_nodes = tune_get(TMDNET_TUNE_ET_BOTH_MAX_NODES);
+  if (acc & TMDNET_ET_PREACT) {
+    if (!dr || gpk || gpv) return kBadArgument;
+    if (n < fuse_nodes) return et_launch<T, 13, false>(V, A, st);
+    if ((rc = et_launch<T, 11, false>(V, A, st))) return rc;
+    return et_launch<T, 12, false>(V, A, st);
+  }
   const bool ag = !dr && (acc & TMDNET_ACC_GRADS) && (A.pk || A.pv);
   static const int merged = getenv("TMDNET_ET_MERGED") ? atoi(getenv("TMDNET_ET_MERGED")) : 1;
   const int merged_min = tune_get(TMDNET_TUNE_ET_MERGED_MIN_NODES);
diff --git a/torchmd-net_amd/csrc/gemm.hip b/torchmd-net_amd/csrc/gemm.hip
--- a/torchmd-net_amd/csrc/gemm.hip
+++ b/torchmd-net_amd/csrc/gemm.hip
@@ -739,6 +739,119 @@
     for (int mb = 0; mb < MB; ++mb) {
       const int m = m0 + 16 * mb + (lane & 15);
       if (m < P.M) *reinterpret_cast<f4*>(P.C + (size_t)m * P.ldc + n0 + nl) = acc[mb] + bv;
+    }
+  }
+}
+
+struct ActArgs {
+  Args p;
+  const float* dA;
+  float* D;
+  int act;
+};
+
+template <int KS, int MB, int BN, bool DER>
+__global__ __launch_bounds__(256) void k_proj_act_x3(ActArgs Q) {
+  const Args& P = Q.p;
+  constexpr int K = 32 * KS, LD = K + 8;
+  __shared__ __attribute__((aligned(16))) unsigned short w[3][BN][LD];
+  __shared__ __attribute__((aligned(16))) float sb[BN];
+  const int lane = threadIdx.x & 63, wave = threadIdx.x >> 6;
+  const int n0 = blockIdx.x * BN;
+  const int m0 = (blockIdx.y * 4 + wave) * (16 * MB);
+  const int nr = min(BN, P.N - n0);
+  const int kq = 8 * (lane >> 4);
+  constexpr int ND = DER ? 2 : 1;
+  float4 ar[ND][MB][KS][2];
+#pragma unroll
+  for (int mb = 0; mb < MB; ++mb) {
+    const size_t ro = (size_t)min(m0 + 16 * mb + (lane & 15), P.M - 1) * P.lda + kq;
+#pragma unroll
+    for (int ks = 0; ks < KS; ++ks) {
+      ar[0][mb][ks][0] = *reinterpret_cast<const float4*>(P.A + ro + 32 * ks);
+      ar[0][mb][ks][1] = *reinterpret_cast<const float4*>(P.A + ro + 32 * ks + 4);
+      if constexpr (DER) {
+        ar[1][mb][ks][0] = *reinterpret_cast<const float4*>(Q.dA + ro + 32 * ks);
+        ar[1][mb][ks][1] = *reinterpret_cast<const float4*>(Q.dA + ro + 32 * ks + 4);
+      }
+    }
+  }
+  constexpr int CH = K / 8;
+  constexpr int NL = (3 * BN * CH + 255) / 256;
+  u4 stg[NL];
+#pragma unroll
+  for (int i = 0; i < NL; ++i) {
+    const int c = threadIdx.x + 256 * i;
+    const int p = c / (BN * CH), rc = c % (BN * CH), n = rc / CH, k = (rc % CH) * 8;
+    if (c < 3 * BN * CH)
+      stg[i] = *reinterpret_cast<const u4*>(P.Wp + p * P.pstride + (size_t)min(n0 + n, P.N - 1) * K + k);
+  }
+#pragma unroll
+  for (int i = 0; i < NL; ++i) {
+    const int c = threadIdx.x + 256 * i;
+    const int p = c / (BN * CH), rc = c % (BN * CH), n = rc / CH, k = (rc % CH) * 8;
+    if (c < 3 * BN * CH) *reinterpret_cast<u4*>(&w[p][n][k]) = stg[i];
+  }
+  if (threadIdx.x < BN) sb[threadIdx.x] = P.bias ? P.bias[min(n0 + (int)threadIdx.x, P.N - 1)] : 0.f;
+  bf8 a[ND][MB][KS][3];
+#pragma unroll
+  for (int d = 0; d < ND; ++d)
+#pragma unroll
+    for (int mb = 0; mb < MB; ++mb)
+#pragma unroll
+      for (int ks = 0; ks < KS; ++ks) split8(ar[d][mb][ks][0], ar[d][mb][ks][1], a[d][mb][ks]);
+  __syncthreads();
+  if (m0 >= P.M) return;
+  const int code = Q.act;
+  for (int nb = 0; nb < nr; nb += 16) {
+    bf8 b[KS][3];
+#pragma unroll
+    for (int ks = 0; ks < KS; ++ks)
+#pragma unroll
+      for (int p = 0; p < 3; ++p)
+        b[ks][p] = *reinterpret_cast<const bf8*>(&w[p][nb + (lane & 15)][32 * ks + kq]);
+    f4 acc[ND][MB];
+#pragma unroll
+    for (int d = 0; d < ND; ++d)
+#pragma unroll
+      for (int mb = 0; mb < MB; ++mb) acc[d][mb] = f4{0.f, 0.f, 0.f, 0.f};
+    constexpr int TW[6] = {2, 1, 0, 1, 0, 0}, TA[6] = {0, 1, 2, 0, 1, 0};
+#pragma unroll
+    for (int t = 0; t < 6; ++t)
+#pragma unroll
+      for (int ks = 0; ks < KS; ++ks)
+#pragma unroll
+        for (int mb = 0; mb < MB; ++mb)
+#pragma unroll
+          for (int d = 0; d < ND; ++d)
+            acc[d][mb] = __builtin_amdgcn_mfma_f32_16x16x32_bf16(b[ks][TW[t]], a[d][mb][ks][TA[t]], acc[d][mb], 0, 0, 0);
+    const int nl = nb + 4 * (lane >> 4);
+    const f4 bv = *reinterpret_cast<const f4*>(&sb[nl]);
+#pragma unroll
+    for (int mb = 0; mb < MB; ++mb) {
+      const int m = m0 + 16 * mb + (lane & 15);
+      const f4 pre = acc[0][mb] + bv;
+      f4 s, ds;
+      if (code == kActSilu) {
+#pragma unroll
+        for (int i = 0; i < 4; ++i) {
+          const Silu<float> f(pre[i]);
+          s[i] = f.s;
+          ds[i] = DER ? f.d(pre[i]) : 0.f;
+        }
+      } else {
+#pragma unroll
+        for (int i = 0; i < 4; ++i) {
+          const ActF<float> f(pre[i], code);
+          s[i] = f.s;
+          ds[i] = DER ? f.d(pre[i]) : 0.f;
+        }
+      }
+      if (m < P.M) {
+        const size_t o = (size_t)m * P.ldc + n0 + nl;
+        *reinterpret_cast<f4*>(P.C + o) = s;
+        if constexpr (DER) *reinterpret_cast<f4*>(Q.D + o) = ds * acc[1][mb];
+      }
     }
   }
 }
@@ -1682,6 +1795,37 @@
     if (mb == 4) TMD_PROJ(1, 4, 64); else TMD_PROJ(1, 2, 64);
   }
 #undef TMD_PROJ
+  return hipGetLastError() == hipSuccess ? kOk : kLaunchFailed;
+}
+
+extern "C" int tmdnet_proj_act_f32(int M, int N, int K, const void* A, const void* dA, int lda, const void* Wp,
+                                   long long piece_stride, const void* bias, int act, void* S, void* D, int ldc,
+                                   void* stream) {
+  if (M < 0 || N <= 0 || K <= 0 || !A || !Wp || !S || act < kActSilu || act > kActSigmoid) return kBadArgument;
+  if (D && !dA) return kBadArgument;
+  if (M == 0) return kOk;
+  if ((K != 32 && K != 64) || N % 16 || lda < K || ldc < N || lda % 4 || ldc % 4 || piece_stride < (long long)N * K)
+    return kUnsupported;
+  if ((((uintptr_t)A) | ((uintptr_t)dA) | ((uintptr_t)Wp) | ((uintptr_t)S) | ((uintptr_t)D) | ((uintptr_t)bias)) & 15)
+    return kUnsupported;
+  const bool der = D != nullptr;
+  const bool big = M >= 65536 && K == 64 && !der;
+  const int bn = big ? 128 : 64, mb = big ? 4 : 2;
+  proj::ActArgs Q{{M, N, lda, ldc, piece_stride, (const float*)A, (const unsigned short*)Wp, (const float*)bias,
+                   (float*)S},
+                  (const float*)dA, (float*)D, act};
+  const dim3 g((N + bn - 1) / bn, (M + 64 * mb - 1) / (64 * mb));
+  hipStream_t st = (hipStream_t)stream;
+#define TMD_PROJ_ACT(KS_, MB_, BN_, DER_) \
+  hipLaunchKernelGGL((proj::k_proj_act_x3<KS_, MB_, BN_, DER_>), g, dim3(256), 0, st, Q)
+  if (K == 64) {
+    if (big) TMD_PROJ_ACT(2, 4, 128, false);
+    else if (der) TMD_PROJ_ACT(2, 2, 64, true);
+    else TMD_PROJ_ACT(2, 2, 64, false);
+  } else {
+    if (der) TMD_PROJ_ACT(1, 2, 64, true); else TMD_PROJ_ACT(1, 2, 64, false);
+  }
+#undef TMD_PROJ_ACT
   return hipGetLastError() == hipSuccess ? kOk : kLaunchFailed;
 }
 
diff --git a/torchmd-net_amd/torchmdnet/_native.py b/torchmd-net_amd/torchmdnet/_native.py
--- a/torchmd-net_amd/torchmdnet/_native.py
+++ b/torchmd-net_amd/torchmdnet/_native.py
@@ -14,6 +14,7 @@
 ET_V_PLANAR = 4
 BWD2_ACC_EDGE, BWD2_ACC_GVEC = 8, 16
 ET_TWO_PASS = 64
+ET_PREACT = 128
 
 _STATUS = {1: "bad argument", 2: "unsupported configuration", 3: "kernel launch failed",
            4: "workspace too small"}
@@ -122,6 +123,7 @@
     "tmdnet_fep_frags_bytes": (SZ, [ctypes.c_longlong, I]),
     "tmdnet_fep_frags_f32": (I, [ctypes.c_longlong, I, P, P, P, D, D, I, P, P, P]),
     "tmdnet_proj_f32": (I, [I, I, I, P, I, P, ctypes.c_longlong, P, P, I, P]),
+    "tmdnet_proj_act_f32": (I, [I, I, I, P, P, I, P, ctypes.c_longlong, P, I, P, P, I, P]),
     "tmdnet_mse2_fwd": (I, [I, I, P, P, D, I, P, P, D, P, P]),
     "tmdnet_mse2_bwd": (I, [I, I, P, P, D, I, P, P, D, P, P, P, P]),
     "tmdnet_build_info": (ctypes.c_char_p, []),
diff --git a/torchmd-net_amd/torchmdnet/et_stack.py b/torchmd-net_amd/torchmdnet/et_stack.py
--- a/torchmd-net_amd/torchmdnet/et_stack.py
+++ b/torchmd-net_amd/torchmdnet/et_stack.py
@@ -84,6 +84,7 @@
 FEP_BWD = os.environ.get("TMDNET_FEP_BWD", "fused")
 FUSED_BWD = FEP_BWD == "fused"
 DR_MODE = os.environ.get("TMDNET_DR", "auto")
+PREACT = os.environ.get("TMDNET_ET_PREACT", "1") not in ("0", "off")
 SECOND_ORDER = os.environ.get("TMDNET_ET_SECOND_ORDER", "hand")
 RECORD_IN_FORCE_PASS = os.environ.get("TMDNET_ET_RECORD", "1") not in ("0", "off")
 _EXPECT_SECOND_ORDER = [False]
@@ -169,6 +170,8 @@
         self.fep = False
         self.fep_imgs = None
         self.grad_mode = True
+        self.pre = None
+        self.r_grad = True
 
     def split(self, params):
         return [params[i * self.np:(i + 1) * self.np] for i in range(self.n_layers)]
@@ -308,7 +311,7 @@
 
 def _act_pkv(meta, acts, l, f):
     a = acts[l]
-    if a[7] is None and meta.fep_imgs is not None and meta.D:
+    if a[7] is None and (meta.fep_imgs is not None or meta.pre is not None) and meta.D:
         if meta.batched:
             pkv_all, D = meta.dkv_proj(_pair_f(meta, f)), meta.D
             for j in range(meta.n_layers):
@@ -329,7 +332,18 @@
     if not fep:
         meta.fep_imgs = None
     fp = _pair_f(meta, f) if (D and not fep) else f
-    pkv_all = meta.dkv_proj(fp) if (meta.batched and D and not fep) else None
+    meta.pre = None
+    if (PREACT and D and not fep and meta.batched and meta.rbf is not None and r is not None
+            and meta.pairs is not None and x.is_cuda and x.dtype == torch.float32 and fp.shape[0] > 0
+            and (not want_bwd or (meta.r_grad and not _EXPECT_SECOND_ORDER[0]))):
+        fdp = None
+        if want_bwd:
+            fdp = meta.fdp_pairs
+            if fdp is None:
+                fdp = kernels.rbf_deriv(r, *meta.rbf, rows=meta.pairs[1])
+        meta.pre = kernels.proj_act(fp, fdp, meta.dkv_eff[0], meta.dkv_eff[1], (meta.acts >> 8) & 15,
+                                    wp=meta.dkv_split())
+    pkv_all = meta.dkv_proj(fp) if (meta.batched and D and not fep and meta.pre is None) else None
     layers = meta.split(params)
     L = len(layers)
     od = dict(dtype=x.dtype, device=x.device)
@@ -368,14 +382,18 @@
                                         meta.fep_imgs[l], meta.fep_frag, meta.graph, meta.heads, xa, veca,
                                         flags=meta.flags)
         else:
-            if pkv_all is not None:
-                pkv = pkv_all[:, l * D:(l + 1) * D]
+            flags = meta.flags
+            if meta.pre is not None:
+                pkv, rows = None, meta.pre[0][:, l * D:(l + 1) * D]
+                flags |= nat.ET_PREACT
+            elif pkv_all is not None:
+                pkv = rows = pkv_all[:, l * D:(l + 1) * D]
             else:
-                pkv = meta.dkv_proj(fp, l) if dkv_w is not None else None
-            pk = pkv[:, :H] if meta.hk else None
-            pv = pkv[:, H * int(meta.hk):] if meta.hv else None
+                pkv = rows = meta.dkv_proj(fp, l) if dkv_w is not None else None
+            pk = rows[:, :H] if meta.hk else None
+            pv = rows[:, H * int(meta.hk):] if meta.hv else None
             kernels.et_message_fwd_launch(qkv[:, :H], qkv[:, H:2 * H], qkv[:, 2 * H:], vec, pk, pv, C, u,
-                                          meta.graph, meta.heads, xa, veca, meta.flags, meta.pk_rows)
+                                          meta.graph, meta.heads, xa, veca, flags, meta.pk_rows)
         if nf and l + 1 < len(layers):
             o, x_next, vec_next = _oproj_epi(xa, o_w, o_b, x, vec, vecp, veca, vec_all[l + 1])
             acts.append((x, vec, xn, mean, rstd, qkv, vecp, pkv, xa, o))
@@ -418,10 +436,12 @@
     g_r = None
     fused = (dr and meta.fep and not rec and not inj and meta.fep_imgs is not None and FUSED_BWD
              and all(a[7] is None for a in acts[:meta.n_layers]))
+    pre = (dr and not fused and not rec and not inj and meta.pre is not None and meta.pre[1] is not None
+           and all(a[7] is None for a in acts[:meta.n_layers]))
     if dr:
         assert has_e and not any(need_ws) and meta.rbf is not None
         g_r = zbuf[4 * E:]
-        if not fused:
+        if not fused and not pre:
             if meta.fdp_pairs is not None and meta.pairs is not None:
                 fdp = meta.fdp_pairs
             else:
@@ -471,15 +491,18 @@
         gX = gX + x_top
     for l in reversed(range(meta.n_layers)):
         p = layers[l]
-        x, vec, xn, mean, rstd, qkv, vecp, pkv, xa, o_ = acts[l] if fused else _act_pkv(meta, acts, l, f)
+        x, vec, xn, mean, rstd, qkv, vecp, pkv, xa, o_ = acts[l] if (fused or pre) else _act_pkv(meta, acts, l, f)
         ln_w, ln_b = p[0], p[1]
         vec_w, o_w = p[8], p[9]
         qkv_w, _ = meta.qkv_eff[l]
         dkv_w, _ = meta.dkv_layer(l)
         g_qkv, g_o, g_vecp = g_qkv_all[l], g_o_all[l], g_vecp_all[l]
         gpk = gpv = dpk = dpv = None
+        if pre:
+            pkv, dpkv = meta.pre[0][:, l * D:(l + 1) * D], meta.pre[1][:, l * D:(l + 1) * D]
+        elif dr and not fused:
+            dpkv = dpkv_all[:, l * D:(l + 1) * D] if meta.batched else meta.dkv_proj(fdp, l, bias=False)
         if dr and not fused:
-            dpkv = dpkv_all[:, l * D:(l + 1) * D] if meta.batched else meta.dkv_proj(fdp, l, bias=False)
             dpk = dpkv[:, :H] if meta.hk else None
             dpv = dpkv[:, H * int(meta.hk):] if meta.hv else None
         if has_e and (not dr or rec):
@@ -505,7 +528,7 @@
         if acc and vec is not None:
             g_vec_in = injected("vec", l) if injected("vec", l) is not None else torch.zeros((N, 3, H), **o)
         flags = (nat.ACC_VEC_RESIDUAL | (nat.ACC_EDGE if l < L - 1 else 0) | meta.flags
-                 | (nat.ACC_GRADS if acc else 0))
+                 | (nat.ACC_GRADS if acc else 0) | (nat.ET_PREACT if pre else 0))
         if fused:
             kernels.et_fused_bwd_launch(qkv[:, :H], qkv[:, H:2 * H], qkv[:, 2 * H:], vec, C, u, meta.fep_imgs[l],
                                         meta.fep_frag, graph, meta.heads, g_xa, gV, g_qkv[:, :H], g_qkv[:, H:2 * H],
@@ -1045,6 +1068,7 @@
     @staticmethod
     def forward(ctx, meta, x, f, C, u, r, *params):
         want = meta.grad_mode and any(ctx.needs_input_grad)
+        meta.r_grad = bool(r is not None and ctx.needs_input_grad[5])
         x_out, vec_out, acts = _forward_layers(meta, x, f, C, u, params, r=r, want_bwd=want)
         ctx.meta = meta
         ctx.acts = acts
diff --git a/torchmd-net_amd/torchmdnet/kernels.py b/torchmd-net_amd/torchmdnet/kernels.py
--- a/torchmd-net_amd/torchmdnet/kernels.py
+++ b/torchmd-net_amd/torchmdnet/kernels.py
@@ -1427,6 +1427,35 @@
                 nat.check(rc, "tmdnet_proj_f32")
                 return out
     return gemm_lib(Gemm(A, W, True, bias, out, False))
+
+
+def proj_act(A, dA, W, bias, act, wp=None, row0=0, out=None):
+    M, K = A.shape
+    N = W.shape[0]
+    if not (PROJ == "x3" and A.is_cuda and A.dtype == torch.float32 and A.stride(1) == 1 and M > 0
+            and (bias is None or (bias.is_contiguous() and bias.dtype == torch.float32))
+            and (dA is None or (dA.is_cuda and dA.dtype == torch.float32 and dA.shape == A.shape
+                                and dA.stride(1) == 1 and dA.stride(0) == A.stride(0)))):
+        return None
+    if wp is None:
+        wp, row0 = proj_split(W), 0
+    if wp is None:
+        return None
+    if out is not None:
+        S, D = out
+        if S.stride(1) != 1 or (D is not None and (D.stride(1) != 1 or D.stride(0) != S.stride(0))):
+            return None
+    else:
+        S = torch.empty((M, N), dtype=A.dtype, device=A.device)
+        D = torch.empty((M, N), dtype=A.dtype, device=A.device) if dA is not None else None
+    rc = nat.load().tmdnet_proj_act_f32(M, N, K, A.data_ptr(), None if dA is None else dA.data_ptr(), A.stride(0),
+                                        wp[0, row0:].data_ptr(), wp.shape[1] * K,
+                                        None if bias is None else bias.data_ptr(), int(act), S.data_ptr(),
+                                        None if D is None else D.data_ptr(), S.stride(0), nat.stream(A.device))
+    if rc == GEMM_UNSUPPORTED:
+        return None
+    nat.check(rc, "tmdnet_proj_act_f32")
+    return S, D
 
 
 def wgrad_tn(problems):
```
